# Windere/EAS-SNN

Measured on AMD Instinct MI355X. Metric: event-frames/sec (T=3) SYOLOX-S Gen1 304x240, higher is better.
Workload: dtype f32

## Files before the change

eas_snn_amd/_ctx.py:

```python
import os


def _env_flag(name, default='1'):
    return os.environ.get(name, default) == '1'


class Context:
    def __init__(self):
        self.spike_planes = _env_flag('EAS_SPIKE_PLANES')
        self.conv_stats = _env_flag('EAS_CONV_STATS')
        self.conv_stats_max_blocks = int(os.environ.get('EAS_CONV_STATS_MAX_BLOCKS', '4096'))
        self.fused_eval = {'1': 'all', 'all': 'all', '0': False, 'auto': 'auto'}.get(os.environ.get('EAS_FUSED_EVAL', 'auto'), 'auto')
        self.fused_ann_eval = _env_flag('EAS_FUSED_ANN_EVAL')
        self.arsnn_fused = _env_flag('EAS_ARSNN_FUSED')
        self.small_dgrad = os.environ.get('EAS_SMALL_DGRAD', '1') != '0'
        self.defer_wgrad_reduce = _env_flag('EAS_DEFER_WGRAD_REDUCE', '0')
        self.wgrad_side_batch = int(os.environ.get('EAS_WGRAD_SIDE', '16'))
        self.dwconv = _env_flag('EAS_DWCONV')
        self.device_ap = _env_flag('EAS_DEVICE_AP')
        self.verify_small_int = False
        self.state_writeback = True
        self.planes_scope = False
        self.invstd_scope = None
        self.want_conv_stats = False
        self.conv_stats_slot = None
        self.replicas = 1
        self.pack_scope = None
        self.pack_gen = 0
        self.frozen = None
        self.pending_reduce = []
        self.side = {'stream': None, 'pending': [], 'keep': [], 'dirty': False}
        self.deferred_counters = None
        self.call_log = None
        self.timer = None
        self.tag = None
        self.conv_sink = None


ctx = Context()
```

eas_snn_amd/_lib.py:

```python
import ctypes as C
import os
import subprocess

_HERE = os.path.dirname(os.path.abspath(__file__))
LIB_PATH = os.environ.get('EAS_LIB') or os.path.join(_HERE, 'libeas_hip.so')
CSRC = os.path.join(_HERE, 'csrc')

_lib = None

_f32p, _i32p, _u32p, _u16p, _u8p, _i64p, _f64p = (C.c_void_p,) * 7
_P = C.c_void_p

class EasWgradReduceJob(C.Structure):
    _fields_ = [('slabs', C.c_void_p), ('grad_w', C.c_void_p), ('n', C.c_int), ('slabs_count', C.c_int)]


class EasSmallconvPackJob(C.Structure):
    _fields_ = [('w', C.c_void_p), ('wr', C.c_void_p), ('Cin', C.c_int), ('Cout', C.c_int), ('k', C.c_int), ('mode', C.c_int),
                ('o_total', C.c_int), ('o_off', C.c_int)]


class EasBnPending(C.Structure):
    _fields_ = [('partial', C.c_void_p), ('chunks', C.c_int), ('replicas', C.c_int), ('count', C.c_double), ('eps', C.c_float),
                ('momentum', C.c_float), ('running_mean', C.c_void_p), ('running_var', C.c_void_p), ('pitch', C.c_int)]


class EasLifRange(C.Structure):
    _fields_ = [('gamma', C.c_void_p), ('beta', C.c_void_p), ('mean', C.c_void_p), ('invstd', C.c_void_p), ('w_logit', C.c_void_p),
                ('k_const', C.c_float), ('v_th', C.c_float), ('planes', C.c_void_p), ('out_f32', C.c_void_p), ('out_ctot', C.c_int),
                ('out_c0', C.c_int), ('res_planes', C.c_void_p), ('res_f32', C.c_void_p), ('res_ctot', C.c_int), ('rate', C.c_void_p),
                ('v_in', C.c_void_p), ('v_out', C.c_void_p)]


class EasConvBnLifEval(C.Structure):
    _fields_ = [('x', C.c_void_p), ('packed_w', C.c_void_p), ('x_terms', C.c_int), ('x_shared', C.c_int), ('T', C.c_int), ('N', C.c_int),
                ('Cin', C.c_int), ('Cout', C.c_int), ('Hi', C.c_int), ('Wi', C.c_int), ('ksize', C.c_int), ('stride', C.c_int),
                ('csplit', C.c_int), ('range', EasLifRange * 2)]


class EasBnActRange(C.Structure):
    _fields_ = [('gamma', C.c_void_p), ('beta', C.c_void_p), ('mean', C.c_void_p), ('invstd', C.c_void_p), ('out', C.c_void_p),
                ('out_ctot', C.c_int), ('out_c0', C.c_int)]


class EasConvBnActEval(C.Structure):
    _fields_ = [('x', C.c_void_p), ('packed_w', C.c_void_p), ('x_terms', C.c_int), ('NI', C.c_int), ('Cin', C.c_int), ('Cout', C.c_int),
                ('Hi', C.c_int), ('Wi', C.c_int), ('ksize', C.c_int), ('stride', C.c_int), ('act', C.c_int), ('csplit', C.c_int),
                ('range', EasBnActRange * 2)]


class EasConvProblem(C.Structure):
    _fields_ = [('x', C.c_void_p), ('packed_w', C.c_void_p), ('bias', C.c_void_p), ('y', C.c_void_p), ('stats', C.c_void_p),
                ('NI', C.c_int), ('Cin', C.c_int), ('Cout', C.c_int), ('Hi', C.c_int), ('Wi', C.c_int), ('accumulate', C.c_int)]


class EasBnSiluFwdProblem(C.Structure):
    _fields_ = [('y', C.c_void_p), ('mean', C.c_void_p), ('invstd', C.c_void_p), ('gamma', C.c_void_p), ('beta', C.c_void_p),
                ('out', C.c_void_p), ('N', C.c_int), ('C', C.c_int), ('HW', C.c_int), ('out_ctot', C.c_int), ('y_ctot', C.c_int),
                ('pending', EasBnPending)]


class EasBnSiluBwdProblem(C.Structure):
    _fields_ = [('grad_out', C.c_void_p), ('y', C.c_void_p), ('mean', C.c_void_p), ('invstd', C.c_void_p), ('gamma', C.c_void_p),
                ('beta', C.c_void_p), ('grad_y', C.c_void_p), ('grad_gamma', C.c_void_p), ('grad_beta', C.c_void_p),
                ('workspace', C.c_void_p), ('batch_stats', C.c_int), ('N', C.c_int), ('C', C.c_int), ('HW', C.c_int),
                ('grad_out_ctot', C.c_int), ('y_ctot', C.c_int)]


class EasWgradProblem(C.Structure):
    _fields_ = [('x', C.c_void_p), ('grad_y', C.c_void_p), ('workspace', C.c_void_p), ('NI', C.c_int), ('Cin', C.c_int), ('Cout', C.c_int),
                ('Hi', C.c_int), ('Wi', C.c_int)]


class EasChannelSumProblem(C.Structure):
    _fields_ = [('g', C.c_void_p), ('out', C.c_void_p), ('N', C.c_int), ('C', C.c_int), ('HW', C.c_int)]


class EasPredDgradProblem(C.Structure):
    _fields_ = [('gy_a', C.c_void_p), ('w_a', C.c_void_p), ('Ka', C.c_int), ('gy_b', C.c_void_p), ('w_b', C.c_void_p), ('Kb', C.c_int),
                ('gx', C.c_void_p), ('N', C.c_int), ('C', C.c_int), ('HW', C.c_int)]


class EasAdamHyper(C.Structure):
    _fields_ = [('beta1', C.c_double), ('beta2', C.c_double), ('eps', C.c_double), ('group_lr', C.c_double * 16), ('ema_updates', C.c_void_p),
                ('ema_decay', C.c_double), ('ema_ramp', C.c_double)]


ABI_VERSION = 9

PROTOTYPES = {
    'eas_abi_version': (C.c_int, []),
    'eas_kernel_trace_begin': (None, []),
    'eas_kernel_trace_dump': (C.c_int64, [C.c_char_p, C.c_int64]),
    'eas_launch_counter': (C.c_int64, []),
    'eas_status_string': (C.c_char_p, [C.c_int]),
    'eas_conv_bn_lif_eval': (C.c_int, [C.POINTER(EasConvBnLifEval), _P]),
    'eas_conv_bn_lif_eval_supported': (C.c_int, [C.c_int] * 10),
    'eas_conv_bn_act_eval': (C.c_int, [C.POINTER(EasConvBnActEval), _P, _P]),
    'eas_conv_bn_act_eval_group': (C.c_int, [C.POINTER(EasConvBnActEval), C.c_int, _P]),
    'eas_event_histogram': (C.c_int, [_P, _P, _P, _P, C.c_int64, _P, C.c_int, C.c_int, C.c_int, C.c_int, _P, _P, _P]),
    'eas_event_histogram_dat': (C.c_int, [_P, C.c_int64, _P, C.c_int, C.c_int, C.c_int, C.c_int, _P, _P, _P]),
    'eas_counts_to_canvas': (C.c_int, [_P, C.c_int64, C.c_int, C.c_int, C.c_int, C.c_int, _P, _P]),
    'eas_event_voxel_cube': (C.c_int, [_P, _P, _P, _P, C.c_int64, _P, C.c_int, C.c_int, C.c_int, C.c_int, C.c_int, _P, _P]),
    'eas_event_time_surface': (C.c_int, [_P, _P, _P, _P, C.c_int64, _P, C.c_int, C.c_int, C.c_int, C.c_int, C.c_double, _P, _P, _P]),
    'eas_spike_sop_workspace_doubles': (C.c_int64, []),
    'eas_spike_sop': (C.c_int, [_P, C.c_int64, C.c_int, C.c_int, C.c_int, C.c_int, C.c_int, C.c_int, _P, _P, _P]),
    'eas_counts_letterbox': (C.c_int, [_P, _P, C.c_int, C.c_int, C.c_int, C.c_int, C.c_int, C.c_int, _P, _P]),
    'eas_postprocess_workspace_bytes': (C.c_int64, [C.c_int, C.c_int]),
    'eas_postprocess': (C.c_int, [_P, C.c_int, C.c_int, C.c_int, C.c_float, C.c_float, C.c_int, _P, _P, _P, _P]),
    'eas_event_frames': (C.c_int, [_P, _P, _P, _P, C.c_int64, _P, C.c_int, C.c_int, C.c_int, C.c_int, C.c_int, C.c_int, _P, _P, _P, _P]),
    'eas_simota_assign': (C.c_int, [_P] * 8 + [C.c_int] * 4 + [_P] * 4),
    'eas_simota_assign_rows': (C.c_int, [_P] * 6 + [C.c_int] * 4 + [_P] * 4),
    'eas_det_decode': (C.c_int, [C.c_int, _P, _P, _P, _P, _P, C.c_int, C.c_int, _P, _P]),
    'eas_det_decode_eval': (C.c_int, [C.c_int, _P, _P, _P, _P, _P, C.c_int, C.c_int, _P, _P]),
    'eas_det_labels': (C.c_int, [_P, C.c_int, C.c_int, _P, _P, _P, _P, _P]),
    'eas_det_loss_workspace_doubles': (C.c_int64, []),
    'eas_det_loss': (C.c_int, [C.c_int] + [_P] * 8 + [C.c_int, C.c_int] + [_P] * 3 + [C.c_int] + [_P] * 4 + [C.c_int, _P, _P, _P]),
    'eas_upcat_fwd': (C.c_int, [_P, _P, _P, C.c_int64] + [C.c_int] * 5 + [_P]),
    'eas_upcat_bwd': (C.c_int, [_P, _P, _P, C.c_int64] + [C.c_int] * 5 + [_P]),
    'eas_upcat_planes_fwd': (C.c_int, [_P, _P, _P, C.c_int64] + [C.c_int] * 5 + [_P]),
    'eas_focus': (C.c_int, [_P, _P, C.c_int64, C.c_int, C.c_int, C.c_int, C.c_int, _P]),
    'eas_event_voxel_grid': (C.c_int, [_P, _P, _P, _P, C.c_int64, _P, C.c_int, C.c_int, C.c_int, C.c_int, _P, _P]),
    'eas_event_window_search': (C.c_int, [_P, _P, C.c_int, _P, _P, C.c_int, C.c_int64, C.c_int64, C.c_int, _P, _P]),
    'eas_event_histogram_dat_ranges': (C.c_int, [_P, _P] + [C.c_int] * 4 + [_P, _P, _P]),
    'eas_stacked_hist_event_sum': (C.c_int, [_P, _P] + [C.c_int] * 7 + [_P, _P]),
    'eas_lif_fwd': (C.c_int, [_P, _P, _P, _P, C.c_float, C.c_float, C.c_float, C.c_int, _P, _P, _P, C.c_int, C.c_int64, _P]),
    'eas_lif_bwd': (C.c_int, [_P, _P, _P, _P, _P, _P, C.c_float, C.c_float, C.c_float, C.c_int, C.c_int, C.c_float,
                              _P, _P, _P, C.c_int, C.c_int64, _P]),
    'eas_lif_bwd_patan': (C.c_int, [_P, _P, _P, _P, _P, _P, C.c_float, C.c_float, C.c_float, C.c_int, _P, _P,
                                    _P, _P, _P, C.c_int, C.c_int64, _P]),
    'eas_reduce_workspace_floats': (C.c_int64, [C.c_int64]),
    'eas_time_mean': (C.c_int, [_P, _P, C.c_int, C.c_int64, _P]),
    'eas_channel_sum': (C.c_int, [_P, _P, C.c_int, C.c_int, C.c_int, _P]),
    'eas_bn_stats': (C.c_int, [_P, C.c_int, C.c_int, C.c_int, C.c_int, C.c_float, C.c_float, _P, _P, _P, _P, _P, _P]),
    'eas_bn_workspace_doubles': (C.c_int64, [C.c_int]),
    'eas_bn_lif_fwd': (C.c_int, [_P, _P, _P, _P, _P, _P, _P, _P, C.c_float, C.c_float, C.c_float, C.c_int, _P, _P,
                                 C.c_int, C.c_int, C.c_int, C.c_int, C.c_int, _P]),
    'eas_bn_lif_bwd': (C.c_int, [_P, _P, _P, _P, _P, _P, _P, _P, _P, C.c_float, C.c_float, C.c_float, C.c_int, C.c_int,
                                 C.c_float, C.c_int, _P, _P, _P, _P, _P, C.c_int, C.c_int, C.c_int, C.c_int, C.c_int, _P]),
    'eas_bn_silu_fwd': (C.c_int, [_P] * 6 + [C.c_int] * 3 + [_P]),
    'eas_bn_silu_fwd_ex': (C.c_int, [_P] * 6 + [C.c_int] * 3 + [C.POINTER(EasBnPending), C.c_int, C.c_int, _P]),
    'eas_bn_stats_partial': (C.c_int, [_P, C.c_int, C.c_int, C.c_int, C.c_int, _P, _P]),
    'eas_bn_lif_fwd_ex': (C.c_int, [_P, C.c_int, _P, _P, _P, _P, _P, _P, _P, C.c_float, C.c_float, C.c_float, C.c_int, _P, _P,
                                    C.c_int, C.c_int, C.c_int, C.c_int, C.c_int, C.POINTER(EasBnPending), _P, C.c_int, _P, _P, C.c_int, _P]),
    'eas_bn_lif_bwd_ex': (C.c_int, [_P, C.c_int, _P, _P, C.c_int, _P, _P, _P, _P, _P, _P, C.c_float, C.c_float, C.c_float, C.c_int, C.c_int,
                                    C.c_float, C.c_int, _P, _P, _P, _P, _P, C.c_int, C.c_int, C.c_int, C.c_int, C.c_int, _P]),
    'eas_bn_lif_bwd_patan': (C.c_int, [_P, C.c_int, _P, _P, C.c_int, _P, _P, _P, _P, _P, _P, C.c_float, C.c_float, C.c_float, C.c_int, _P,
                                       _P, C.c_int, _P, _P, _P, _P, _P, C.c_int, C.c_int, C.c_int, C.c_int, C.c_int, _P]),
    'eas_bn_silu_bwd': (C.c_int, [_P] * 6 + [C.c_int] + [_P] * 4 + [C.c_int] * 5 + [_P]),
    'eas_arsnn_step_fwd': (C.c_int, [_P] * 14 + [C.c_int, C.c_int, C.c_int, C.c_int, C.c_float, C.c_float, C.c_int,
                                                 C.c_int, C.c_int, C.c_int, _P]),
    'eas_arsnn_step_bwd': (C.c_int, [_P] * 13 + [C.c_int, C.c_int, C.c_int, C.c_int, C.c_float, C.c_float, C.c_int,
                                                 C.c_float, C.c_int, C.c_int, C.c_int, _P]),
    'eas_arsnn_tail_fwd': (C.c_int, [_P] * 6 + [C.c_int] * 7 + [_P]),
    'eas_arsnn_tail_bwd': (C.c_int, [_P] * 6 + [C.c_int] * 7 + [_P]),
    'eas_arsnn_fused_step_fwd': (C.c_int, [_P] * 19 + [C.c_int, C.c_int, C.c_int, C.c_int, C.c_float, C.c_float, C.c_int,
                                                       C.c_int, C.c_int, C.c_int, C.c_int, _P]),
    'eas_smallconv_packed_floats': (C.c_int64, [C.c_int] * 3),
    'eas_smallconv_pack_weights': (C.c_int, [_P, C.c_int, _P]),
    'eas_smallconv_bwd_input_dual': (C.c_int, [_P] * 6 + [C.c_int] * 4 + [_P]),
    'eas_smallconv_fwd': (C.c_int, [_P] * 4 + [C.c_int] * 8 + [_P]),
    'eas_smallconv_bwd_input': (C.c_int, [_P] * 4 + [C.c_int] * 6 + [_P]),
    'eas_smallconv_bwd_weight': (C.c_int, [_P] * 5 + [C.c_int] * 7 + [_P]),
    'eas_smallconv_wgrad_workspace_floats': (C.c_int64, [C.c_int] * 3),
    'eas_conv_packed_weight_bytes': (C.c_int64, [C.c_int] * 4),
    'eas_conv_pack_weights': (C.c_int, [_P, _P] + [C.c_int] * 4 + [_P]),
    'eas_conv_pack_weights_many': (C.c_int, [_P, C.c_int, _P]),
    'eas_conv_fwd_supported': (C.c_int, [C.c_int] * 8),
    'eas_conv_wgrad_parts': (C.c_int, [C.c_int] * 7),
    'eas_conv_fwd': (C.c_int, [_P] * 4 + [C.c_int] * 8 + [_P, _P]),
    'eas_conv_fwd_act': (C.c_int, [_P] * 4 + [C.c_int] * 9 + [_P, _P]),
    'eas_conv_fwd_planes': (C.c_int, [_P] * 4 + [C.c_int] * 7 + [_P, C.c_int, _P]),
    'eas_spike_planes_from_f32': (C.c_int, [_P, C.c_int, _P, C.c_int, C.c_int64, C.c_int, C.c_int, _P, _P]),
    'eas_spike_planes_to_f32': (C.c_int, [_P, C.c_int, _P, C.c_int, C.c_int64, C.c_int, C.c_int, _P]),
    'eas_conv_fwd_stats': (C.c_int, [_P] * 3 + [C.c_int] * 8 + [_P, _P, C.c_int, _P]),
    'eas_conv_fwd_stats_blocks': (C.c_int, [C.c_int] * 8),
    'eas_conv_dgrad_s2': (C.c_int, [_P] * 3 + [C.c_int] * 5 + [_P]),
    'eas_conv_dgrad_small_supported': (C.c_int, [C.c_int] * 5),
    'eas_conv_dgrad_small': (C.c_int, [_P] * 3 + [C.c_int] * 5 + [_P]),
    'eas_conv_wgrad_workspace_floats': (C.c_int64, [C.c_int] * 8),
    'eas_conv_wgrad': (C.c_int, [_P] * 4 + [C.c_int] * 8 + [_P]),
    'eas_conv_wgrad_partial': (C.c_int, [_P] * 3 + [C.c_int] * 8 + [_P]),
    'eas_conv_wgrad_planes_partial': (C.c_int, [_P] * 3 + [C.c_int] * 7 + [_P]),
    'eas_conv_wgrad_reduce_many': (C.c_int, [_P, C.c_int, _P]),
    'eas_dwconv_supported': (C.c_int, [C.c_int] * 6),
    'eas_dwconv_fwd_stats_blocks': (C.c_int, [C.c_int] * 6),
    'eas_dwconv_fwd': (C.c_int, [_P] * 4 + [C.c_int] * 5 + [_P, C.c_int, _P]),
    'eas_dwconv_fwd_planes': (C.c_int, [_P] * 4 + [C.c_int] * 5 + [_P, C.c_int, _P]),
    'eas_dwconv_dgrad': (C.c_int, [_P] * 3 + [C.c_int] * 5 + [_P]),
    'eas_dwconv_wgrad_workspace_floats': (C.c_int64, [C.c_int] * 5),
    'eas_dwconv_wgrad': (C.c_int, [_P] * 4 + [C.c_int] * 5 + [_P]),
    'eas_dwconv_wgrad_planes': (C.c_int, [_P] * 4 + [C.c_int] * 5 + [_P]),
    'eas_spp_pool_fwd': (C.c_int, [_P, _P, C.c_int64] + [C.c_int] * 6 + [_P]),
    'eas_spp_pool_bwd': (C.c_int, [_P, _P, _P, C.c_int64] + [C.c_int] * 6 + [_P]),
    'eas_spp_pool_planes_fwd': (C.c_int, [_P, _P, C.c_int64] + [C.c_int] * 6 + [_P]),
    'eas_spp_pool_planes_bwd': (C.c_int, [_P, _P, _P, C.c_int64] + [C.c_int] * 6 + [_P]),
    'eas_conv_fwd_group_plan': (C.c_int, [C.POINTER(EasConvProblem), C.c_int, C.c_int, C.c_int, C.POINTER(C.c_int)]),
    'eas_conv_fwd_group': (C.c_int, [C.POINTER(EasConvProblem), C.c_int, C.c_int, C.c_int, _P]),
    'eas_bn_silu_fwd_group': (C.c_int, [C.POINTER(EasBnSiluFwdProblem), C.c_int, _P]),
    'eas_bn_silu_bwd_group': (C.c_int, [C.POINTER(EasBnSiluBwdProblem), C.c_int, _P]),
    'eas_conv_wgrad_group_plan': (C.c_int, [C.POINTER(EasWgradProblem), C.c_int, C.c_int, C.c_int, C.POINTER(C.c_int)]),
    'eas_conv_wgrad_group_partial': (C.c_int, [C.POINTER(EasWgradProblem), C.c_int, C.c_int, C.c_int, _P]),
    'eas_channel_sum_group': (C.c_int, [C.POINTER(EasChannelSumProblem), C.c_int, _P]),
    'eas_pred_dgrad_group': (C.c_int, [C.POINTER(EasPredDgradProblem), C.c_int, _P]),
    'eas_adam_table_entry_bytes': (C.c_int, []),
    'eas_adam_chunk': (C.c_int, []),
    'eas_adam_step': (C.c_int, [_P, C.c_int, C.c_longlong, C.c_double, C.c_double, C.c_double, _P]),
    'eas_adam_advance_steps': (C.c_int, [_P, C.c_int, _P]),
    'eas_adam_step_ex': (C.c_int, [_P, C.c_int, C.c_longlong, C.POINTER(EasAdamHyper), _P]),
    'eas_adam_advance_steps_ex': (C.c_int, [_P, C.c_int, _P, _P]),
    'eas_cocoeval_supported': (C.c_int, [C.c_int64] * 3 + [C.c_int] * 5 + [C.c_int64]),
    'eas_cocoeval_workspace_bytes': (C.c_int64, [C.c_int64]),
    'eas_cocoeval_keys': (C.c_int, [_P, _P, _P, C.c_int64, _P, _P, C.c_int64, C.c_int64, C.c_int, _P, _P, _P]),
    'eas_cocoeval_match': (C.c_int, [_P, _P, _P, C.c_int64, _P, _P, _P, _P, C.c_int64, C.c_int64, C.c_int, _P, C.c_int, _P, C.c_int, C.c_int,
                                     C.c_int64, _P, _P, _P, _P, _P, _P]),
    'eas_cocoeval_accumulate': (C.c_int, [_P] * 5 + [C.c_int64, _P, C.c_int, C.c_int, _P, C.c_int, C.c_int, _P, C.c_int, _P, _P, _P, _P]),
}


class EasHipError(RuntimeError):
    pass


def build(verbose=False):
    cmd = ['make', '-C', CSRC, '-j', str(min(8, os.cpu_count() or 1))]
    r = subprocess.run(cmd, stdout=subprocess.PIPE, stderr=subprocess.STDOUT, text=True)
    if verbose or r.returncode != 0:
        print(r.stdout)
    if r.returncode != 0:
        raise EasHipError('building libeas_hip.so failed')
    return LIB_PATH


def _bind_host_hip_runtime():
    import torch
    cand = os.path.join(os.path.dirname(torch.__file__), 'lib', 'libamdhip64.so')
    if not os.path.exists(cand):
        cand = 'libamdhip64.so'
    C.CDLL(cand, mode=C.RTLD_GLOBAL)


_PRIVATE_STREAMS = []


def private_stream():
    import torch
    _bind_host_hip_runtime()
    rt = C.CDLL(None)
    handle = C.c_void_p()
    rc = rt.hipStreamCreateWithFlags(C.byref(handle), C.c_uint(1))
    if rc != 0 or not handle.value:
        raise EasHipError(f'hipStreamCreateWithFlags failed ({rc})')
    st = torch.cuda.ExternalStream(handle.value)
    _PRIVATE_STREAMS.append(st)
    return st


def lib():
    global _lib
    if _lib is None:
        if not os.path.exists(LIB_PATH):
            raise EasHipError(
                f'{LIB_PATH} is missing: the HIP extension has not been built and eas_snn_amd has no CPU fallback. '
                'Run `python -c "import __graft_entry__ as g; g.build()"`.')
        _bind_host_hip_runtime()
        handle = C.CDLL(LIB_PATH)
        for name, (res, args) in PROTOTYPES.items():
            fn = getattr(handle, name)
            fn.restype = res
            fn.argtypes = args
        if handle.eas_abi_version() != ABI_VERSION:
            raise EasHipError('libeas_hip.so ABI version mismatch; rebuild')
        _lib = handle
    return _lib


def check(status, what):
    if status != 0:
        msg = lib().eas_status_string(status).decode()
        raise EasHipError(f'{what}: status {status} ({msg})')


def ptr(t):
    return None if t is None else t.data_ptr()


_RAW_STREAM = None


def stream():
    global _RAW_STREAM
    if _RAW_STREAM is None:
        import torch
        raw = getattr(torch._C, '_cuda_getCurrentRawStream', None)
        if raw is not None:
            _RAW_STREAM = lambda: raw(torch.cuda.current_device())
        else:
            _RAW_STREAM = lambda: torch.cuda.current_stream().cuda_stream
    return _RAW_STREAM()
```

eas_snn_amd/csrc/arsnn.hip:

```cpp
#include "eas_common.h"
#include "smallconv_core.h"

namespace {

constexpr int VEC = 4;

typedef int8_t eas_state_t;
__device__ __forceinline__ int4 load_q8(const eas_state_t* p) {
    const int w = *reinterpret_cast<const int*>(p);
    return make_int4((int)(int8_t)(w & 0xFF), (int)(int8_t)((w >> 8) & 0xFF), (int)(int8_t)((w >> 16) & 0xFF), (int)(int8_t)((w >> 24) & 0xFF));
}
__device__ __forceinline__ void store_q8(eas_state_t* p, const int4& v) {
    *reinterpret_cast<int*>(p) = (v.x & 0xFF) | ((v.y & 0xFF) << 8) | ((v.z & 0xFF) << 16) | ((v.w & 0xFF) << 24);
}

struct StepCfg {
    int t, Ts, readout, spike_attach, soft_reset;
    float thresh, v_reset, sg_alpha;
    int64_t plane;
    int64_t total;
};

__device__ __forceinline__ void step_elem(float g_in, float c_in, float g_rec, float c_rec, float v, float vsum,
                                          int32_t& seg, int32_t& tl, float* __restrict__ agg, int64_t i,
                                          const StepCfg& c, float& v_out, float& vsum_out, float& spike, float& gate,
                                          float& vn) {
    gate = eas_sigmoidf(g_in + g_rec);
    const float cur = c_in + c_rec;
    vn = gate * v + cur;
    spike = (vn - c.thresh) > 0.0f ? 1.0f : 0.0f;
    v_out = c.soft_reset ? vn - c.thresh * spike : vn * (1.0f - spike) + c.v_reset * spike;
    const float vs1 = vsum + vn;
    if (spike != 0.0f) {
        if (c.readout != 3 && seg < c.Ts) {
            float val = c.readout == 0 ? vs1 : (c.readout == 1 ? v_out : vs1 / (float)(c.t - tl));
            if (c.spike_attach) val = val * spike;
            agg[(int64_t)seg * c.total + i] += val;
            seg += 1;
            tl = c.t;
        }
        vsum_out = c.readout == 3 ? vs1 : 0.0f;
    } else {
        vsum_out = vs1;
    }
}

__global__ __launch_bounds__(EAS_BLOCK) void arsnn_step_fwd_kernel(
    const float* __restrict__ conv_in, const float* __restrict__ conv_rec, const float* __restrict__ v,
    const float* __restrict__ vsum, eas_state_t* __restrict__ seg, eas_state_t* __restrict__ t_last, float* __restrict__ agg,
    float* __restrict__ v_out, float* __restrict__ vsum_out, float* __restrict__ spike_out,
    float* __restrict__ gate_save, float* __restrict__ vn_save, eas_state_t* __restrict__ seg_before,
    eas_state_t* __restrict__ tl_before, StepCfg c) {
    const int64_t ngroups = c.total / VEC;
    for (int64_t g = (int64_t)blockIdx.x * blockDim.x + threadIdx.x; g < ngroups; g += (int64_t)gridDim.x * blockDim.x) {
        const int64_t i = g * VEC;
        const int64_t n = i / c.plane;
        const int64_t r = i - n * c.plane;
        const int64_t cb = n * 2 * c.plane + r;
        const float4 gi = *reinterpret_cast<const float4*>(conv_in + cb);
        const float4 ci = *reinterpret_cast<const float4*>(conv_in + cb + c.plane);
        const float4 gr = *reinterpret_cast<const float4*>(conv_rec + cb);
        const float4 cr = *reinterpret_cast<const float4*>(conv_rec + cb + c.plane);
        float4 vv = make_float4(0.f, 0.f, 0.f, 0.f), vs = vv;
        int4 sg = make_int4(0, 0, 0, 0), tl = make_int4(-1, -1, -1, -1);
        if (v) {
            vv = *reinterpret_cast<const float4*>(v + i);
            vs = *reinterpret_cast<const float4*>(vsum + i);
            sg = load_q8(seg + i);
            tl = load_q8(t_last + i);
        }
        if (seg_before) store_q8(seg_before + i, sg);
        if (tl_before) store_q8(tl_before + i, tl);
        float4 vo, vso, sp, ga, vn;
        step_elem(gi.x, ci.x, gr.x, cr.x, vv.x, vs.x, sg.x, tl.x, agg, i + 0, c, vo.x, vso.x, sp.x, ga.x, vn.x);
        step_elem(gi.y, ci.y, gr.y, cr.y, vv.y, vs.y, sg.y, tl.y, agg, i + 1, c, vo.y, vso.y, sp.y, ga.y, vn.y);
        step_elem(gi.z, ci.z, gr.z, cr.z, vv.z, vs.z, sg.z, tl.z, agg, i + 2, c, vo.z, vso.z, sp.z, ga.z, vn.z);
        step_elem(gi.w, ci.w, gr.w, cr.w, vv.w, vs.w, sg.w, tl.w, agg, i + 3, c, vo.w, vso.w, sp.w, ga.w, vn.w);
        *reinterpret_cast<float4*>(v_out + i) = vo;
        *reinterpret_cast<float4*>(vsum_out + i) = vso;
        *reinterpret_cast<float4*>(spike_out + i) = sp;
        store_q8(seg + i, sg);
        store_q8(t_last + i, tl);
        if (gate_save) *reinterpret_cast<float4*>(gate_save + i) = ga;
        if (vn_save) *reinterpret_cast<float4*>(vn_save + i) = vn;
    }
}

template <int K, bool HAS_G>
__global__ __launch_bounds__(NT, 2) void arsnn_fused_step_fwd_kernel(
    const float* __restrict__ a_in, const float* __restrict__ wr_in, const float* __restrict__ b_in, const float* __restrict__ a_g,
    const float* __restrict__ wr_g, const float* __restrict__ b_g, const float* __restrict__ r_const, const float* __restrict__ v,
    const float* __restrict__ vsum, eas_state_t* __restrict__ seg, eas_state_t* __restrict__ t_last, float* __restrict__ agg,
    float* __restrict__ v_out, float* __restrict__ vsum_out, float* __restrict__ spike_out, float* __restrict__ gate_save,
    float* __restrict__ vn_save, eas_state_t* __restrict__ seg_before, eas_state_t* __restrict__ tl_before, StepCfg c, int N, int H, int W) {
    using SG = Stage<4, K, true>;
    constexpr int LWF = SG::PITCH, PLANE = SG::PLANE;
    using St = typename SG::St;
    St st;
    st.init(H, W);
    __shared__ __attribute__((aligned(16))) float lds[4 * PLANE];
    const int tiles_x = (W + TW - 1) / TW, tiles_y = (H + TH - 1) / TH;
    const int ntiles = N * tiles_x * tiles_y;
    const int tx = threadIdx.x & 15, ty = threadIdx.x >> 4;
    const int HW = H * W;
    float4 pre[St::PER];
    unsigned okm = 0;
    int tile = blockIdx.x;
    if (tile < ntiles)
        okm = st.load(a_in, pre, tile / (tiles_x * tiles_y), H, W, ((tile / tiles_x) % tiles_y) * TH, (tile % tiles_x) * TW);
    for (; tile < ntiles; tile += gridDim.x) {
        const int n = tile / (tiles_x * tiles_y);
        const int ty0 = ((tile / tiles_x) % tiles_y) * TH, tx0 = (tile % tiles_x) * TW;
        const int nxt = tile + gridDim.x;
        __syncthreads();
        st.store(lds, pre, okm);
        __syncthreads();
        if (HAS_G) okm = st.load(a_g, pre, n, H, W, ty0, tx0);
        else if (nxt < ntiles) okm = st.load(a_in, pre, nxt / (tiles_x * tiles_y), H, W, ((nxt / tiles_x) % tiles_y) * TH, (nxt % tiles_x) * TW);
        const int oy = ty0 + ty, ox = tx0 + 4 * tx;
        const bool inside = oy < H && ox < W;
        const int pix = oy * W + ox;
        float4 vv[2], vs[2], rg[2], rcur[2];
        int4 sg[2], tl[2];
#pragma unroll
        for (int c2 = 0; c2 < 2; ++c2) {
            vv[c2] = make_float4(0.f, 0.f, 0.f, 0.f); vs[c2] = vv[c2]; rg[c2] = vv[c2]; rcur[c2] = vv[c2];
            sg[c2] = make_int4(0, 0, 0, 0); tl[c2] = make_int4(-1, -1, -1, -1);
            if (inside) {
                const int64_t i = ((int64_t)n * 2 + c2) * HW + pix;
                if (v) {
                    vv[c2] = *reinterpret_cast<const float4*>(v + i);
                    vs[c2] = *reinterpret_cast<const float4*>(vsum + i);
                    sg[c2] = load_q8(seg + i);
                    tl[c2] = load_q8(t_last + i);
                }
                if (!HAS_G && r_const) {
                    rg[c2] = *reinterpret_cast<const float4*>(r_const + (int64_t)c2 * HW + pix);
                    rcur[c2] = *reinterpret_cast<const float4*>(r_const + (int64_t)(2 + c2) * HW + pix);
                }
            }
        }
        __builtin_amdgcn_sched_barrier(0);
        f2 X[4][2], R[4][2];
#pragma unroll
        for (int op = 0; op < 2; ++op) {
            const f2 bx = b_in ? f2{b_in[2 * op], b_in[2 * op + 1]} : f2{0.f, 0.f};
            const f2 bg = (HAS_G && b_g) ? f2{b_g[2 * op], b_g[2 * op + 1]} : f2{0.f, 0.f};
#pragma unroll
            for (int j = 0; j < 4; ++j) { X[j][op] = bx; R[j][op] = bg; }
        }
        sc_accumulate<4, 4, K, LWF, SG::NQ, SG::OFS>(lds, PLANE, wr_in, X, tx, ty);
        if (HAS_G) {
            __syncthreads();
            st.store(lds, pre, okm);
            __syncthreads();
            if (nxt < ntiles) okm = st.load(a_in, pre, nxt / (tiles_x * tiles_y), H, W, ((nxt / tiles_x) % tiles_y) * TH, (nxt % tiles_x) * TW);
            sc_accumulate<4, 4, K, LWF, SG::NQ, SG::OFS>(lds, PLANE, wr_g, R, tx, ty);
        }
        if (inside) {
#pragma unroll
            for (int c2 = 0; c2 < 2; ++c2) {
                float gi[4], ci[4], gr[4], cr[4];
#pragma unroll
                for (int j = 0; j < 4; ++j) {
                    gi[j] = c2 ? X[j][0].y : X[j][0].x;
                    ci[j] = c2 ? X[j][1].y : X[j][1].x;
                    gr[j] = c2 ? R[j][0].y : R[j][0].x;
                    cr[j] = c2 ? R[j][1].y : R[j][1].x;
                }
                if (!HAS_G && r_const) {
                    gr[0] = rg[c2].x; gr[1] = rg[c2].y; gr[2] = rg[c2].z; gr[3] = rg[c2].w;
                    cr[0] = rcur[c2].x; cr[1] = rcur[c2].y; cr[2] = rcur[c2].z; cr[3] = rcur[c2].w;
                }
                const int64_t i = ((int64_t)n * 2 + c2) * HW + pix;
                if (seg_before) store_q8(seg_before + i, sg[c2]);
                if (tl_before) store_q8(tl_before + i, tl[c2]);
                float4 vo, vso, sp, ga, vn;
                step_elem(gi[0], ci[0], gr[0], cr[0], vv[c2].x, vs[c2].x, sg[c2].x, tl[c2].x, agg, i + 0, c, vo.x, vso.x, sp.x, ga.x, vn.x);
                step_elem(gi[1], ci[1], gr[1], cr[1], vv[c2].y, vs[c2].y, sg[c2].y, tl[c2].y, agg, i + 1, c, vo.y, vso.y, sp.y, ga.y, vn.y);
                step_elem(gi[2], ci[2], gr[2], cr[2], vv[c2].z, vs[c2].z, sg[c2].z, tl[c2].z, agg, i + 2, c, vo.z, vso.z, sp.z, ga.z, vn.z);
                step_elem(gi[3], ci[3], gr[3], cr[3], vv[c2].w, vs[c2].w, sg[c2].w, tl[c2].w, agg, i + 3, c, vo.w, vso.w, sp.w, ga.w, vn.w);
                *reinterpret_cast<float4*>(v_out + i) = vo;
                *reinterpret_cast<float4*>(vsum_out + i) = vso;
                *reinterpret_cast<float4*>(spike_out + i) = sp;
                store_q8(seg + i, sg[c2]);
                store_q8(t_last + i, tl[c2]);
                if (gate_save) *reinterpret_cast<float4*>(gate_save + i) = ga;
                if (vn_save) *reinterpret_cast<float4*>(vn_save + i) = vn;
            }
        }
    }
}

__device__ __forceinline__ void step_elem_bwd(float gv_out, float gvs_out, float gsp, const float* __restrict__ g_agg,
                                              int64_t i, float v_prev, float vsum_prev, float gate, float vn, int32_t seg_b,
                                              int32_t tl_b, const StepCfg& c, float& g_gatepre, float& g_cur,
                                              float& g_v_prev, float& g_vsum_prev) {
    const float spike = (vn - c.thresh) > 0.0f ? 1.0f : 0.0f;
    const bool fired = spike != 0.0f;
    const float vs1 = vsum_prev + vn;
    float d_vs1 = (fired && c.readout != 3) ? 0.0f : gvs_out;
    float d_vout = gv_out;
    float d_s = gsp;
    if (fired && c.readout != 3 && seg_b < c.Ts) {
        const float ga = g_agg[(int64_t)seg_b * c.total + i];
        float d_pre = ga;
        if (c.spike_attach) {
            const float v_out = c.soft_reset ? vn - c.thresh : c.v_reset;
            const float pre = c.readout == 0 ? vs1 : (c.readout == 1 ? v_out : vs1 / (float)(c.t - tl_b));
            d_s += ga * pre;
            d_pre = ga * spike;
        }
        if (c.readout == 0) d_vs1 += d_pre;
        else if (c.readout == 1) d_vout += d_pre;
        else d_vs1 += d_pre / (float)(c.t - tl_b);
    }
    float d_vn = d_vs1;
    g_vsum_prev = d_vs1;
    if (c.soft_reset) {
        d_vn += d_vout;
        d_s += d_vout * (-c.thresh);
    } else {
        d_vn += d_vout * (1.0f - spike);
        d_s += d_vout * (c.v_reset - vn);
    }
    d_vn += d_s * eas_surrogate_grad(EAS_SG_RECT, c.sg_alpha, vn - c.thresh);
    g_cur = d_vn;
    g_v_prev = d_vn * gate;
    g_gatepre = (d_vn * v_prev) * gate * (1.0f - gate);
}

__global__ __launch_bounds__(EAS_BLOCK) void arsnn_step_bwd_kernel(
    const float* __restrict__ g_v_out, const float* __restrict__ g_vsum_out, const float* __restrict__ g_spike,
    const float* __restrict__ g_agg, const float* __restrict__ v_prev, const float* __restrict__ vsum_prev,
    const float* __restrict__ gate_save, const float* __restrict__ vn_save, const eas_state_t* __restrict__ seg_before,
    const eas_state_t* __restrict__ tl_before, float* __restrict__ g_conv, float* __restrict__ g_v_prev,
    float* __restrict__ g_vsum_prev, StepCfg c) {
    for (int64_t i = (int64_t)blockIdx.x * blockDim.x + threadIdx.x; i < c.total; i += (int64_t)gridDim.x * blockDim.x) {
        const int64_t n = i / c.plane;
        const int64_t r = i - n * c.plane;
        const int64_t cb = n * 2 * c.plane + r;
        float gg, gc, gvp, gvsp;
        step_elem_bwd(g_v_out ? g_v_out[i] : 0.f, g_vsum_out ? g_vsum_out[i] : 0.f, g_spike ? g_spike[i] : 0.f, g_agg, i,
                      v_prev ? v_prev[i] : 0.f, vsum_prev ? vsum_prev[i] : 0.f, gate_save[i], vn_save[i], seg_before[i], tl_before[i], c, gg, gc,
                      gvp, gvsp);
        g_conv[cb] = gg;
        g_conv[cb + c.plane] = gc;
        g_v_prev[i] = gvp;
        g_vsum_prev[i] = gvsp;
    }
}

__global__ __launch_bounds__(EAS_BLOCK) void arsnn_tail_fwd_kernel(const float* __restrict__ v, const float* __restrict__ vsum,
                                                                   const float* __restrict__ spike_last,
                                                                   const eas_state_t* __restrict__ seg,
                                                                   const eas_state_t* __restrict__ t_last, float* __restrict__ agg,
                                                                   int Tm, int Ts, int readout, int write_zero, int64_t total) {
    for (int64_t i = (int64_t)blockIdx.x * blockDim.x + threadIdx.x; i < total; i += (int64_t)gridDim.x * blockDim.x) {
        if (spike_last[i] != 0.0f) continue;
        const int s = seg[i];
        if (s >= Ts) continue;
        float val = readout == 0 ? vsum[i] : (readout == 1 ? v[i] : vsum[i] / (float)(Tm - 1 - t_last[i]));
        if (write_zero) val = val * 0.0f;
        agg[(int64_t)s * total + i] += val;
    }
}

__global__ __launch_bounds__(EAS_BLOCK) void arsnn_tail_bwd_kernel(const float* __restrict__ g_agg,
                                                                   const float* __restrict__ spike_last,
                                                                   const eas_state_t* __restrict__ seg,
                                                                   const eas_state_t* __restrict__ t_last, float* __restrict__ g_v,
                                                                   float* __restrict__ g_vsum, int Tm, int Ts, int readout,
                                                                   int write_zero, int64_t total) {
    for (int64_t i = (int64_t)blockIdx.x * blockDim.x + threadIdx.x; i < total; i += (int64_t)gridDim.x * blockDim.x) {
        float gv = 0.f, gvs = 0.f;
        const int s = seg[i];
        if (spike_last[i] == 0.0f && s < Ts && !write_zero) {
            const float ga = g_agg[(int64_t)s * total + i];
            if (readout == 0) gvs = ga;
            else if (readout == 1) gv = ga;
            else gvs = ga / (float)(Tm - 1 - t_last[i]);
        }
        g_v[i] = gv;
        g_vsum[i] = gvs;
    }
}

}

extern "C" {

int eas_arsnn_step_fwd(const float* conv_in, const float* conv_rec, const float* v, const float* vsum,
                       int8_t* seg, int8_t* t_last, float* agg, float* v_out, float* vsum_out, float* spike_out,
                       float* gate_save, float* vn_save, int8_t* seg_before, int8_t* t_last_before, int t,
                       int Ts, int readout, int spike_attach, float thresh, float v_reset, int soft_reset, int N,
                       int C2, int HW, eas_stream_t stream) {
    if (!conv_in || !conv_rec || (v == nullptr) != (vsum == nullptr) || !seg || !t_last || !agg || !v_out || !vsum_out || !spike_out)
        return EAS_ERR_INVALID_ARG;
    if (N < 1 || C2 < 1 || HW < 1 || Ts < 1 || t < 0 || readout < 0 || readout > 3) return EAS_ERR_INVALID_ARG;
    if (HW % VEC != 0 || Ts > 127 || t > 126) return EAS_ERR_UNSUPPORTED;
    if (((uintptr_t)conv_in | (uintptr_t)conv_rec | (uintptr_t)v | (uintptr_t)vsum | (uintptr_t)seg | (uintptr_t)t_last |
         (uintptr_t)v_out | (uintptr_t)vsum_out | (uintptr_t)spike_out | (uintptr_t)gate_save | (uintptr_t)vn_save |
         (uintptr_t)seg_before | (uintptr_t)t_last_before) & 15)
        return EAS_ERR_INVALID_ARG;
    StepCfg c{t, Ts, readout, spike_attach, soft_reset, thresh, v_reset, 1.0f, (int64_t)C2 * HW, (int64_t)N * C2 * HW};
    EAS_CLEAR_ERR();
    EAS_LAUNCH(arsnn_step_fwd_kernel, dim3(eas_grid_1d(c.total / VEC)), dim3(EAS_BLOCK), 0, eas_s(stream), conv_in,
                       conv_rec, v, vsum, seg, t_last, agg, v_out, vsum_out, spike_out, gate_save, vn_save, seg_before,
                       t_last_before, c);
    EAS_CHECK_LAUNCH();
    return EAS_OK;
}

int eas_arsnn_fused_step_fwd(const float* a_in, const float* wr_in, const float* b_in, const float* a_g, const float* wr_g, const float* b_g,
                             const float* r_const, const float* v, const float* vsum, int8_t* seg, int8_t* t_last, float* agg, float* v_out,
                             float* vsum_out, float* spike_out, float* gate_save, float* vn_save, int8_t* seg_before, int8_t* t_last_before,
                             int t, int Ts, int readout, int spike_attach, float thresh, float v_reset, int soft_reset, int N, int H, int W, int k,
                             eas_stream_t stream) {
    if (!a_in || !wr_in || (a_g && !wr_g) || (v == nullptr) != (vsum == nullptr) || !seg || !t_last || !agg || !v_out || !vsum_out || !spike_out)
        return EAS_ERR_INVALID_ARG;
    if (N < 1 || H < 1 || W < 1 || Ts < 1 || t < 0 || readout < 0 || readout > 3) return EAS_ERR_INVALID_ARG;
    if (W % 4 != 0 || (k != 3 && k != 5 && k != 7) || Ts > 127 || t > 126) return EAS_ERR_UNSUPPORTED;
    if (((uintptr_t)a_in | (uintptr_t)a_g | (uintptr_t)wr_in | (uintptr_t)wr_g | (uintptr_t)r_const | (uintptr_t)v | (uintptr_t)vsum | (uintptr_t)seg | (uintptr_t)t_last |
         (uintptr_t)v_out | (uintptr_t)vsum_out | (uintptr_t)spike_out | (uintptr_t)gate_save | (uintptr_t)vn_save | (uintptr_t)seg_before |
         (uintptr_t)t_last_before) & 15)
        return EAS_ERR_INVALID_ARG;
    const int HW = H * W;
    StepCfg c{t, Ts, readout, spike_attach, soft_reset, thresh, v_reset, 1.0f, (int64_t)2 * HW, (int64_t)N * 2 * HW};
    int tiles = N * ((H + TH - 1) / TH) * ((W + TW - 1) / TW);
    if (tiles > 256 * 6) tiles = 256 * 6;
    hipStream_t st = eas_s(stream);
    EAS_CLEAR_ERR();
#define EAS_FUSED(K_)                                                                                                                        \
    do {                                                                                                                                     \
        if (a_g)                                                                                                                             \
            EAS_LAUNCH((arsnn_fused_step_fwd_kernel<K_, true>), dim3(tiles), dim3(NT), 0, st, a_in, wr_in, b_in, a_g, wr_g, b_g,     \
                               r_const, v, vsum, seg, t_last, agg, v_out, vsum_out, spike_out, gate_save, vn_save, seg_before,               \
                               t_last_before, c, N, H, W);                                                                                    \
        else                                                                                                                                 \
            EAS_LAUNCH((arsnn_fused_step_fwd_kernel<K_, false>), dim3(tiles), dim3(NT), 0, st, a_in, wr_in, b_in, a_g, wr_g, b_g,    \
                               r_const, v, vsum, seg, t_last, agg, v_out, vsum_out, spike_out, gate_save, vn_save, seg_before,               \
                               t_last_before, c, N, H, W);                                                                                    \
    } while (0)
    if (k == 3) EAS_FUSED(3);
    else if (k == 5) EAS_FUSED(5);
    else EAS_FUSED(7);
#undef EAS_FUSED
    EAS_CHECK_LAUNCH();
    return EAS_OK;
}

int eas_arsnn_step_bwd(const float* g_v_out, const float* g_vsum_out, const float* g_spike, const float* g_agg,
                       const float* v_prev, const float* vsum_prev, const float* gate_save, const float* vn_save,
                       const int8_t* seg_before, const int8_t* t_last_before, float* g_conv, float* g_v_prev,
                       float* g_vsum_prev, int t, int Ts, int readout, int spike_attach, float thresh,
                       float v_reset, int soft_reset, float sg_alpha, int N, int C2, int HW, eas_stream_t stream) {
    if (!g_agg || (v_prev == nullptr) != (vsum_prev == nullptr) || !gate_save || !vn_save || !seg_before || !t_last_before || !g_conv ||
        !g_v_prev || !g_vsum_prev)
        return EAS_ERR_INVALID_ARG;
    if (N < 1 || C2 < 1 || HW < 1 || Ts < 1 || t < 0 || readout < 0 || readout > 3 || !(sg_alpha > 0.f))
        return EAS_ERR_INVALID_ARG;
    StepCfg c{t, Ts, readout, spike_attach, soft_reset, thresh, v_reset, sg_alpha, (int64_t)C2 * HW,
              (int64_t)N * C2 * HW};
    EAS_CLEAR_ERR();
    EAS_LAUNCH(arsnn_step_bwd_kernel, dim3(eas_grid_1d(c.total)), dim3(EAS_BLOCK), 0, eas_s(stream), g_v_out,
                       g_vsum_out, g_spike, g_agg, v_prev, vsum_prev, gate_save, vn_save, seg_before, t_last_before, g_conv,
                       g_v_prev, g_vsum_prev, c);
    EAS_CHECK_LAUNCH();
    return EAS_OK;
}

int eas_arsnn_tail_fwd(const float* v, const float* vsum, const float* spike_last, const int8_t* seg,
                       const int8_t* t_last, float* agg, int Tm, int Ts, int readout, int write_zero, int N,
                       int C2, int HW, eas_stream_t stream) {
    if (!v || !vsum || !spike_last || !seg || !t_last || !agg || N < 1 || C2 < 1 || HW < 1 || Ts < 1 || readout < 0 ||
        readout > 2)
        return EAS_ERR_INVALID_ARG;
    const int64_t total = (int64_t)N * C2 * HW;
    EAS_CLEAR_ERR();
    EAS_LAUNCH(arsnn_tail_fwd_kernel, dim3(eas_grid_1d(total)), dim3(EAS_BLOCK), 0, eas_s(stream), v, vsum,
                       spike_last, seg, t_last, agg, Tm, Ts, readout, write_zero, total);
    EAS_CHECK_LAUNCH();
    return EAS_OK;
}

int eas_arsnn_tail_bwd(const float* g_agg, const float* spike_last, const int8_t* seg, const int8_t* t_last,
                       float* g_v, float* g_vsum, int Tm, int Ts, int readout, int write_zero, int N, int C2,
                       int HW, eas_stream_t stream) {
    if (!g_agg || !spike_last || !seg || !t_last || !g_v || !g_vsum || N < 1 || C2 < 1 || HW < 1 || Ts < 1 ||
        readout < 0 || readout > 2)
        return EAS_ERR_INVALID_ARG;
    const int64_t total = (int64_t)N * C2 * HW;
    EAS_CLEAR_ERR();
    EAS_LAUNCH(arsnn_tail_bwd_kernel, dim3(eas_grid_1d(total)), dim3(EAS_BLOCK), 0, eas_s(stream), g_agg, spike_last,
                       seg, t_last, g_v, g_vsum, Tm, Ts, readout, write_zero, total);
    EAS_CHECK_LAUNCH();
    return EAS_OK;
}

}
```

eas_snn_amd/csrc/smallconv_wgrad_mfma.hip:

```cpp
#include "eas_common.h"

namespace {

typedef __bf16 bf16x8 __attribute__((ext_vector_type(8)));
typedef float f32x16 __attribute__((ext_vector_type(16)));
typedef unsigned int u32x4 __attribute__((ext_vector_type(4)));

constexpr int RB = 8;
constexpr int WC = 64;
constexpr int HALO = 8;
constexpr int XC = WC + 2 * HALO;
constexpr int NTH = 256;
constexpr int NWV = NTH / 64;

template <int CIN, int COUT, int K>
struct Sw {
    static constexpr int PAD = K / 2;
    static constexpr int GR = RB + K - 1;
    static constexpr int GP = WC + 8;
    static constexpr int G_ROWS = GR * COUT;
    static constexpr int G_TERM = G_ROWS * GP * 2;
    static constexpr int XP = XC;
    static constexpr int X_ROWS = RB * CIN;
    static constexpr int X_RAW = (X_ROWS + 1) * XP * 2;
    static constexpr int X_COPY = X_RAW + ((4 + 32 - (X_RAW / 4) % 32) % 32) * 4;
    static constexpr int X_ONES = X_ROWS * XP * 2 + 8;
    static constexpr int X_TERM = 2 * X_COPY;
    static constexpr int G_BYTES = 3 * G_TERM;
    static constexpr int X_BYTES = 3 * X_TERM;
    static constexpr int STAGE_BYTES = G_BYTES + X_BYTES;
    static constexpr int RED_BYTES = 2 * NWV * 32 * 33 * 4;
    static constexpr int LDS_BYTES = STAGE_BYTES > RED_BYTES ? STAGE_BYTES : RED_BYTES;
    static constexpr int NWT = COUT * CIN * K * K;
    static constexpr int NOUT = NWT + COUT;
    static constexpr int G_ITEMS = GR * COUT * (WC / 8);
    static constexpr int X_ITEMS = RB * CIN * (XC / 8);
    static_assert(COUT * K <= 32 && CIN * K + 1 <= 32, "does not fit one 32x32 tile");
    static_assert(PAD + 1 <= HALO && XC <= XP && (X_COPY / 4) % 32 == 4 && X_COPY % 16 == 0, "x staging geometry");
    static_assert(2 * STAGE_BYTES <= 160 * 1024 && STAGE_BYTES % 16 == 0, "LDS");
    static_assert(RB == 2 * NWV, "two rows per wave (4 waves) / one row per wave (8 waves)");
};

__device__ __forceinline__ void sw_split3(float v, __bf16& hi, __bf16& mid, __bf16& lo) {
    hi = (__bf16)v;
    const float r1 = v - (float)hi;
    mid = (__bf16)r1;
    lo = (__bf16)(r1 - (float)mid);
}

template <int O, int NV>
__device__ __forceinline__ void sw_store_terms(unsigned char* dst, int term_stride, const float (&v)[NV]) {
    bf16x8 t0, t1, t2;
#pragma unroll
    for (int j = 0; j < 8; ++j) {
        __bf16 a, b, c;
        sw_split3(v[O + j], a, b, c);
        t0[j] = a;
        t1[j] = b;
        t2[j] = c;
    }
    *(bf16x8*)dst = t0;
    *(bf16x8*)(dst + term_stride) = t1;
    *(bf16x8*)(dst + 2 * term_stride) = t2;
}

template <int NV>
__device__ __forceinline__ void sw_load_row(const float* __restrict__ row, bool row_ok, int c0, int W, float (&v)[NV]) {
#pragma unroll
    for (int j = 0; j < NV; ++j) {
        const int c = c0 + j;
        v[j] = (row_ok && c >= 0 && c < W) ? row[c] : 0.f;
    }
}

template <int CIN, int COUT, int K, bool VEC>
__global__ __launch_bounds__(VEC ? 4 * NTH : NTH) void smallconv_wgrad_mfma_kernel(const float* __restrict__ gy, const float* __restrict__ x,
                                                                                   float* __restrict__ partial, int N, int H, int W, int x_tm) {
    using S = Sw<CIN, COUT, K>;
    const int xS = x_tm ? N / x_tm : 0;
    auto x_img = [&](int n) {
        if (x_tm == 0) return n;
        const int t = n / xS;
        return (n - t * xS) * x_tm + (x_tm - 1 - t);
    };
    constexpr int PAD = S::PAD;
    constexpr int NBUF = VEC ? 2 : 1;
    extern __shared__ __attribute__((aligned(16))) unsigned char smem[];
    const int tid = threadIdx.x, lane = tid & 63;
    constexpr int NTS = VEC ? 2 * NTH : NTH;
    constexpr int NCW = VEC ? 2 * NWV : NWV;
    constexpr int RPW = RB / NCW;
    const int wave = VEC ? (tid >> 6) - NTS / 64 : (tid >> 6);
    const int r = lane & 31, hh = lane >> 5;

    const bool g0 = (r & 3) == r || (r >= 12 && r < 16) || (r >= 20 && r < 28);
    const int ra = r < COUT * K ? r : (g0 ? 0 : 4);
    const int a_kh = ra / COUT, a_co = ra % COUT;
    const int a_off = (((2 * PAD - a_kh) * COUT + a_co) * S::GP + 8 * hh) * 2;
    const int a_rs = COUT * S::GP * 2, a_kss = 32;
    const bool b_ones = r == CIN * K;
    const int rb = r < CIN * K ? r : 0;
    const int b_ci = rb / K, b_kw = rb % K;
    const int sft = b_kw - PAD;
    const int odd = sft & 1;
    const int b_off = b_ones ? S::X_ONES : odd * S::X_COPY + (b_ci * S::XP + HALO + 8 * hh + (sft - odd)) * 2;
    const int b_rs = b_ones ? 0 : CIN * S::XP * 2, b_kss = b_ones ? 0 : 32;

    for (int i = tid; i < NBUF * 3 * 4; i += blockDim.x) {
        const int buf = i / 12, tm = (i % 12) / 4, d = i & 3;
        *(unsigned int*)(smem + buf * S::STAGE_BYTES + S::G_BYTES + tm * S::X_TERM + S::X_ONES + 4 * d) = tm == 0 ? 0x3f803f80u : 0u;
    }

    f32x16 acc0, acc1;
#pragma unroll
    for (int e = 0; e < 16; ++e) {
        acc0[e] = 0.0f;
        acc1[e] = 0.0f;
    }

    const int bands = (H + RB - 1) / RB, chunks = (W + WC - 1) / WC;
    const int ntiles = N * bands * chunks;
    const size_t plane = (size_t)H * W;

    auto tile_origin = [&](int t, int& n, int& h0, int& w0) {
        n = t / (bands * chunks);
        const int rest = t - n * bands * chunks;
        const int band = rest / chunks;
        h0 = band * RB;
        w0 = (rest - band * chunks) * WC;
    };

    struct Frag { bf16x8 a[3], b[3]; };
    const unsigned char* pa0 = smem + a_off + wave * a_rs;
    const unsigned char* pb0 = smem + S::G_BYTES + b_off + wave * b_rs;
    auto read_frag = [&](Frag& f, int step) {
        const int ks = step / RPW, i = step % RPW;
        const unsigned char* pa = pa0 + i * (NCW * a_rs) + ks * a_kss;
        const unsigned char* pb = pb0 + i * (NCW * b_rs) + ks * b_kss;
#pragma unroll
        for (int tm = 0; tm < 3; ++tm) {
            f.a[tm] = *(const bf16x8*)(pa + tm * S::G_TERM);
            const unsigned int* q = (const unsigned int*)(pb + tm * S::X_TERM);
            u32x4 d;
            d[0] = q[0]; d[1] = q[1]; d[2] = q[2]; d[3] = q[3];
            f.b[tm] = __builtin_bit_cast(bf16x8, d);
        }
    };
    auto mul6 = [&](f32x16& acc, const Frag& f) {
        acc = __builtin_amdgcn_mfma_f32_32x32x16_bf16(f.a[2], f.b[0], acc, 0, 0, 0);
        acc = __builtin_amdgcn_mfma_f32_32x32x16_bf16(f.a[0], f.b[2], acc, 0, 0, 0);
        acc = __builtin_amdgcn_mfma_f32_32x32x16_bf16(f.a[1], f.b[1], acc, 0, 0, 0);
        acc = __builtin_amdgcn_mfma_f32_32x32x16_bf16(f.a[1], f.b[0], acc, 0, 0, 0);
        acc = __builtin_amdgcn_mfma_f32_32x32x16_bf16(f.a[0], f.b[1], acc, 0, 0, 0);
        acc = __builtin_amdgcn_mfma_f32_32x32x16_bf16(f.a[0], f.b[0], acc, 0, 0, 0);
    };
    auto compute = [&](int buf) {
        constexpr int STEPS = RPW * (WC / 16);
        pa0 = smem + buf * S::STAGE_BYTES + a_off + wave * a_rs;
        pb0 = smem + buf * S::STAGE_BYTES + S::G_BYTES + b_off + wave * b_rs;
        Frag f0, f1;
        read_frag(f0, 0);
#pragma unroll
        for (int st = 0; st < STEPS; st += 2) {
            read_frag(f1, st + 1);
            mul6(acc0, f0);
            if (st + 2 < STEPS) read_frag(f0, st + 2);
            mul6(acc1, f1);
        }
    };

    auto write_red = [&]() {
        float* red = (float*)smem;
#pragma unroll
        for (int e = 0; e < 16; ++e) {
            const int m = 4 * hh + (e & 3) + 8 * (e >> 2);
            red[(wave * 32 + m) * 33 + r] = acc0[e] + acc1[e];
        }
    };

    if constexpr (VEC) {
        constexpr int NG = (S::G_ITEMS + NTS - 1) / NTS, NX = (S::X_ITEMS + NTS - 1) / NTS;
        int g_dr[NG], g_dc[NG], g_ch[NG], g_lds[NG];
        int x_dr[NX], x_dc[NX], x_ch[NX], x_lds[NX];
        bool g_valid[NG], x_valid[NX];
#pragma unroll
        for (int j = 0; j < NG; ++j) {
            const int id = j * NTS + tid;
            g_valid[j] = tid < NTS && id < S::G_ITEMS;
            const int idc = g_valid[j] ? id : 0;
            const int c8 = idc % (WC / 8), rc = idc / (WC / 8);
            const int co = rc % COUT, jrow = rc / COUT;
            g_dr[j] = jrow - PAD; g_dc[j] = 8 * c8; g_ch[j] = co;
            g_lds[j] = ((jrow * COUT + co) * S::GP + 8 * c8) * 2;
        }
#pragma unroll
        for (int j = 0; j < NX; ++j) {
            const int id = j * NTS + (((j + NG) & 1) ? NTS - 1 - tid : tid);
            x_valid[j] = tid < NTS && id >= 0 && id < S::X_ITEMS;
            const int idc = x_valid[j] ? id : 0;
            const int c8 = idc % (XC / 8), rc = idc / (XC / 8);
            const int ci = rc % CIN, row_l = rc / CIN;
            x_dr[j] = row_l; x_dc[j] = 8 * c8 - HALO; x_ch[j] = ci;
            x_lds[j] = S::G_BYTES + ((row_l * CIN + ci) * S::XP + 8 * c8) * 2;
        }
        struct Pre {
            float4 ga[NG], gb[NG], xa[NX], xb[NX];
            float xc[NX];
            int gm[NG], xm[NX];
        };
        auto issue = [&](Pre& p, int t) {
            int n, h0, w0;
            tile_origin(t, n, h0, w0);
            const int nx = x_img(n);
#pragma unroll
            for (int j = 0; j < NG; ++j) {
                const int row = h0 + g_dr[j], col = w0 + g_dc[j];
                const bool row_ok = g_valid[j] && (unsigned)row < (unsigned)H;
                const bool ok0 = row_ok && col + 4 <= W, ok1 = row_ok && col + 8 <= W;
                const float* prow = gy + ((size_t)n * COUT + g_ch[j]) * plane + (size_t)(row_ok ? row : 0) * W + col;
                p.ga[j] = *(const float4*)(ok0 ? prow : gy);
                p.gb[j] = *(const float4*)(ok1 ? prow + 4 : gy);
                p.gm[j] = (ok0 ? 1 : 0) | (ok1 ? 2 : 0);
            }
#pragma unroll
            for (int j = 0; j < NX; ++j) {
                const int row = h0 + x_dr[j], col = w0 + x_dc[j];
                const bool row_ok = x_valid[j] && row < H;
                const bool ok0 = row_ok && col >= 0 && col + 4 <= W, ok1 = row_ok && col + 4 >= 0 && col + 8 <= W;
                const bool ok2 = row_ok && col + 8 < W;
                const float* prow = x + ((size_t)nx * CIN + x_ch[j]) * plane + (size_t)(row_ok ? row : 0) * W + col;
                p.xa[j] = *(const float4*)(ok0 ? prow : x);
                p.xb[j] = *(const float4*)(ok1 ? prow + 4 : x);
                p.xc[j] = *(ok2 ? prow + 8 : x);
                p.xm[j] = (ok0 ? 1 : 0) | (ok1 ? 2 : 0) | (ok2 ? 4 : 0);
            }
        };
        auto commit = [&](const Pre& p, int buf) {
            unsigned char* const base = smem + buf * S::STAGE_BYTES;
#pragma unroll
            for (int j = 0; j < NG; ++j) {
                if (!g_valid[j]) continue;
                const bool ok0 = p.gm[j] & 1, ok1 = p.gm[j] & 2;
                float v[8];
                v[0] = ok0 ? p.ga[j].x : 0.f; v[1] = ok0 ? p.ga[j].y : 0.f; v[2] = ok0 ? p.ga[j].z : 0.f; v[3] = ok0 ? p.ga[j].w : 0.f;
                v[4] = ok1 ? p.gb[j].x : 0.f; v[5] = ok1 ? p.gb[j].y : 0.f; v[6] = ok1 ? p.gb[j].z : 0.f; v[7] = ok1 ? p.gb[j].w : 0.f;
                sw_store_terms<0, 8>(base + g_lds[j], S::G_TERM, v);
            }
#pragma unroll
            for (int j = 0; j < NX; ++j) {
                if (!x_valid[j]) continue;
                const bool ok0 = p.xm[j] & 1, ok1 = p.xm[j] & 2, ok2 = p.xm[j] & 4;
                float v[9];
                v[0] = ok0 ? p.xa[j].x : 0.f; v[1] = ok0 ? p.xa[j].y : 0.f; v[2] = ok0 ? p.xa[j].z : 0.f; v[3] = ok0 ? p.xa[j].w : 0.f;
                v[4] = ok1 ? p.xb[j].x : 0.f; v[5] = ok1 ? p.xb[j].y : 0.f; v[6] = ok1 ? p.xb[j].z : 0.f; v[7] = ok1 ? p.xb[j].w : 0.f;
                v[8] = ok2 ? p.xc[j] : 0.f;
                unsigned char* dst = base + x_lds[j];
                sw_store_terms<0, 9>(dst, S::X_TERM, v);
                sw_store_terms<1, 9>(dst + S::X_COPY, S::X_TERM, v);
            }
        };
        const int G = gridDim.x;
        const bool stager = __builtin_amdgcn_readfirstlane(tid >> 6) < NTS / 64;
        int t = blockIdx.x;
        if (stager) {
            Pre pa, pb;
            issue(pa, t);
            if (t + G < ntiles) issue(pb, t + G);
            commit(pa, 0);
            if (t + 2 * G < ntiles) issue(pa, t + 2 * G);
            __syncthreads();
            for (;;) {
                if (t + G < ntiles) {
                    commit(pb, 1);
                    if (t + 3 * G < ntiles) issue(pb, t + 3 * G);
                }
                __syncthreads();
                t += G;
                if (t >= ntiles) break;
                if (t + G < ntiles) {
                    commit(pa, 0);
                    if (t + 3 * G < ntiles) issue(pa, t + 3 * G);
                }
                __syncthreads();
                t += G;
                if (t >= ntiles) break;
            }
        } else {
            __syncthreads();
            for (;;) {
                compute(0);
                __syncthreads();
                t += G;
                if (t >= ntiles) break;
                compute(1);
                __syncthreads();
                t += G;
                if (t >= ntiles) break;
            }
            write_red();
        }
    } else {
        __syncthreads();
        for (int t = blockIdx.x; t < ntiles; t += gridDim.x) {
            int n, h0, w0;
            tile_origin(t, n, h0, w0);
            for (int id = tid; id < S::G_ITEMS; id += NTH) {
                const int c8 = id % (WC / 8), rc = id / (WC / 8);
                const int co = rc % COUT, jrow = rc / COUT;
                const int ho = h0 - PAD + jrow;
                const bool row_ok = ho >= 0 && ho < H;
                const float* row = gy + ((size_t)n * COUT + co) * plane + (size_t)(row_ok ? ho : 0) * W;
                float v[8];
                sw_load_row<8>(row, row_ok, w0 + 8 * c8, W, v);
                sw_store_terms<0, 8>(smem + ((jrow * COUT + co) * S::GP + 8 * c8) * 2, S::G_TERM, v);
            }
            for (int id = tid; id < S::X_ITEMS; id += NTH) {
                const int c8 = id % (XC / 8), rc = id / (XC / 8);
                const int ci = rc % CIN, row_l = rc / CIN;
                const int h = h0 + row_l;
                const bool row_ok = h < H;
                const float* row = x + ((size_t)x_img(n) * CIN + ci) * plane + (size_t)(row_ok ? h : 0) * W;
                float v[9];
                sw_load_row<9>(row, row_ok, w0 - HALO + 8 * c8, W, v);
                unsigned char* dst = smem + S::G_BYTES + ((row_l * CIN + ci) * S::XP + 8 * c8) * 2;
                sw_store_terms<0, 9>(dst, S::X_TERM, v);
                sw_store_terms<1, 9>(dst + S::X_COPY, S::X_TERM, v);
            }
            __syncthreads();
            compute(0);
            __syncthreads();
        }
        write_red();
    }

    const float* red = (const float*)smem;
    __syncthreads();
    for (int e = tid; e < S::NOUT; e += blockDim.x) {
        int m, nn;
        if (e < S::NWT) {
            const int co = e / (CIN * K * K), rem = e % (CIN * K * K);
            const int ci = rem / (K * K), kk = rem % (K * K);
            m = (kk / K) * COUT + co;
            nn = ci * K + kk % K;
        } else {
            m = PAD * COUT + (e - S::NWT);
            nn = CIN * K;
        }
        float s = 0.f;
#pragma unroll
        for (int wv = 0; wv < NCW; ++wv) s += red[(wv * 32 + m) * 33 + nn];
        partial[(int64_t)blockIdx.x * S::NOUT + e] = s;
    }
}

template <int CIN, int COUT, int K>
int sw_launch_k(bool vec, const float* gy, const float* x, float* partial, int nblocks, int N, int H, int W, int x_tm, hipStream_t st) {
    using S = Sw<CIN, COUT, K>;
    if (vec) {
        auto kern = smallconv_wgrad_mfma_kernel<CIN, COUT, K, true>;
        static bool attr_set = false;
        if (!attr_set) {
            if (hipFuncSetAttribute((const void*)kern, hipFuncAttributeMaxDynamicSharedMemorySize, 160 * 1024) != hipSuccess) return EAS_ERR_LAUNCH;
            attr_set = true;
        }
        EAS_LAUNCH(kern, dim3(nblocks), dim3(4 * NTH), 2 * S::STAGE_BYTES, st, gy, x, partial, N, H, W, x_tm);
    } else {
        EAS_LAUNCH((smallconv_wgrad_mfma_kernel<CIN, COUT, K, false>), dim3(nblocks), dim3(NTH), S::LDS_BYTES, st, gy, x, partial, N, H, W, x_tm);
    }
    return EAS_OK;
}

template <int CIN, int COUT>
int sw_launch(int k, const float* gy, const float* x, float* partial, int nblocks, int N, int H, int W, int x_tm, hipStream_t st) {
    const bool vec = (W & 3) == 0 && ((((uintptr_t)gy) | ((uintptr_t)x)) & 15) == 0;
    int rc;
    if (vec && nblocks > 256) nblocks = 256;
    switch (k) {
        case 3: rc = sw_launch_k<CIN, COUT, 3>(vec, gy, x, partial, nblocks, N, H, W, x_tm, st); break;
        case 5: rc = sw_launch_k<CIN, COUT, 5>(vec, gy, x, partial, nblocks, N, H, W, x_tm, st); break;
        case 7: rc = sw_launch_k<CIN, COUT, 7>(vec, gy, x, partial, nblocks, N, H, W, x_tm, st); break;
        default: return EAS_ERR_UNSUPPORTED;
    }
    if (rc != EAS_OK) return rc;
    EAS_CHECK_LAUNCH();
    return nblocks;
}

}

int eas_sw_mfma_partials(const float* gy, const float* x, float* partial, int max_blocks, int N, int Cin, int Cout, int H, int W,
                         int k, int x_tm, hipStream_t st) {
    const int64_t tiles = (int64_t)N * ((H + RB - 1) / RB) * ((W + WC - 1) / WC);
    if (tiles > 0x7fffffff) return EAS_ERR_UNSUPPORTED;
    const int nblocks = tiles < max_blocks ? (int)tiles : max_blocks;
    int rc;
    if (Cin == 2 && Cout == 4) rc = sw_launch<2, 4>(k, gy, x, partial, nblocks, N, H, W, x_tm, st);
    else if (Cin == 4 && Cout == 4) rc = sw_launch<4, 4>(k, gy, x, partial, nblocks, N, H, W, x_tm, st);
    else if (Cin == 2 && Cout == 2) rc = sw_launch<2, 2>(k, gy, x, partial, nblocks, N, H, W, x_tm, st);
    else return EAS_ERR_UNSUPPORTED;
    return rc;
}
```

eas_snn_amd/ops.py:

```python
import sys
import types

from . import ops_bn, ops_conv, ops_core, ops_dwconv, ops_lif, ops_sampler
from ._ctx import ctx

_PLUMBING = {'C', 'collections', 'os', 'torch', '_lib', 'check', 'ptr', 'stream', 'opctx'}
for _m in (ops_core, ops_lif, ops_bn, ops_sampler, ops_dwconv, ops_conv):
    for _k, _v in vars(_m).items():
        if not _k.startswith('__') and _k not in _PLUMBING:
            globals()[_k] = _v
from ._lib import check, ptr, stream

from .ops_events import *
from .ops_glue import *
from .ops_det import *

_ALIASES = {
    '_STATE_WRITEBACK': 'state_writeback', '_TIMER': 'timer', '_TAG': 'tag', '_CALL_LOG': 'call_log', 'SPIKE_PLANES': 'spike_planes',
    '_PLANES_SCOPE': 'planes_scope', '_INVSTD_SCOPE': 'invstd_scope', 'CONV_STATS': 'conv_stats', 'CONV_STATS_MAX_BLOCKS': 'conv_stats_max_blocks',
    '_WANT_CONV_STATS': 'want_conv_stats', '_CONV_STATS_SLOT': 'conv_stats_slot', 'FUSED_EVAL': 'fused_eval', '_REPLICAS': 'replicas',
    'ARSNN_FUSED': 'arsnn_fused', 'DEFER_WGRAD_REDUCE': 'defer_wgrad_reduce', '_PENDING_REDUCE': 'pending_reduce',
    'WGRAD_SIDE_BATCH': 'wgrad_side_batch', '_SIDE': 'side',
    'VERIFY_SMALL_INT': 'verify_small_int', 'SMALL_DGRAD': 'small_dgrad', '_PACK_SCOPE': 'pack_scope', '_PACK_GEN': 'pack_gen', '_FROZEN': 'frozen',
    '_CONV_SINK': 'conv_sink', 'FUSED_ANN_EVAL': 'fused_ann_eval', '_DEFERRED': 'deferred_counters', 'DWCONV': 'dwconv',
    'DEVICE_AP': 'device_ap'}


class _OpsModule(types.ModuleType):
    """this module's class: the aliases above as properties, so that ``ops.X`` and ``ops.X = v`` (also ``monkeypatch.setattr(ops, 'X', v)``)
    reach the context object"""


def _alias(field):
    return property(lambda self: getattr(ctx, field), lambda self, value: setattr(ctx, field, value))


for _old, _new in _ALIASES.items():
    assert hasattr(ctx, _new), _new
    setattr(_OpsModule, _old, _alias(_new))
sys.modules[__name__].__class__ = _OpsModule
del _old, _new, _m, _k, _v
```

eas_snn_amd/ops_sampler.py:

```python
import ctypes as C
import os

import torch

from . import _lib
from ._ctx import ctx as opctx
from ._lib import check, ptr, stream
from .ops_core import READOUT_IDS, _call, _dev, _f32c

def smallconv_pack(jobs):
    L = _lib.lib()
    arr = (_lib.EasSmallconvPackJob * len(jobs))()
    outs = []
    for j, (w, mode, o_total, o_off, wr) in enumerate(jobs):
        w = _f32c(w)
        Cout, Cin, k = w.shape[0], w.shape[1], w.shape[-1]
        if wr is None:
            wr = torch.empty(L.eas_smallconv_packed_floats(Cout if mode else Cin, k, o_total), dtype=torch.float32, device=w.device)
        arr[j] = _lib.EasSmallconvPackJob(w.data_ptr(), wr.data_ptr(), Cin, Cout, k, int(mode), int(o_total), int(o_off))
        outs.append(wr)
    check(L.eas_smallconv_pack_weights(arr, len(jobs), stream()), 'eas_smallconv_pack_weights')
    return outs


def smallconv_fwd(x, w, b, relu=False, out=None, wr=None, x_tm=0):
    x = _f32c(x)
    if x_tm:
        assert x.dim() == 5 and x.shape[1] == x_tm
        x = x.view(-1, *x.shape[2:])
    N, Cin, H, W = x.shape
    Cout, k = w.shape[0], w.shape[-1]
    if wr is None:
        wr = smallconv_pack([(w, 0, Cout, 0, None)])[0]
    y = torch.empty((N, Cout, H, W), dtype=torch.float32, device=x.device) if out is None else out
    assert y.is_contiguous() and y.shape == (N, Cout, H, W)
    _call('eas_smallconv_fwd', 4 * (x.numel() + y.numel()), _lib.lib().eas_smallconv_fwd, ptr(x), ptr(wr), ptr(b), ptr(y), N, Cin, Cout,
          H, W, k, int(relu), int(x_tm), stream())
    return y


def smallconv_bwd_input(gy, w, relu_mask=None, out=None, wr=None):
    gy = _f32c(gy)
    N, Cout, H, W = gy.shape
    Cin, k = w.shape[1], w.shape[-1]
    if wr is None:
        wr = smallconv_pack([(w, 1, Cin, 0, None)])[0]
    gx = torch.empty((N, Cin, H, W), dtype=torch.float32, device=gy.device) if out is None else out
    assert gx.is_contiguous() and gx.shape == (N, Cin, H, W)
    _call('eas_smallconv_bwd_input', 4 * (gy.numel() + gx.numel()), _lib.lib().eas_smallconv_bwd_input, ptr(gy), ptr(wr),
          ptr(relu_mask), ptr(gx), N, Cin, Cout, H, W, k, stream())
    return gx


def smallconv_bwd_input_dual(gy, wr8, k, mask_a, mask_b, out_a, out_b):
    gy = _f32c(gy)
    N, C4, H, W = gy.shape
    assert C4 == 4 and out_a.is_contiguous() and out_b.is_contiguous() and out_a.shape == gy.shape == out_b.shape
    _call('eas_smallconv_bwd_input', 4 * 3 * gy.numel(), _lib.lib().eas_smallconv_bwd_input_dual, ptr(gy), ptr(wr8), ptr(mask_a), ptr(mask_b),
          ptr(out_a), ptr(out_b), N, H, W, int(k), stream())


def smallconv_bwd_weight(gy, x, w, x_tm=0):
    gy, x = _f32c(gy), _f32c(x)
    N, Cout, H, W = gy.shape
    assert x.numel() == N * w.shape[1] * H * W and (not x_tm or (x.dim() == 5 and x.shape[1] == x_tm))
    Cin, k = w.shape[1], w.shape[-1]
    L = _lib.lib()
    gw, gb = torch.empty_like(w), torch.empty(Cout, dtype=torch.float32, device=gy.device)
    ws = torch.empty(L.eas_smallconv_wgrad_workspace_floats(Cin, Cout, k), dtype=torch.float32, device=gy.device)
    _call('eas_smallconv_bwd_weight', 4 * (gy.numel() + x.numel()), L.eas_smallconv_bwd_weight, ptr(gy), ptr(x), ptr(gw), ptr(gb),
          ptr(ws), N, Cin, Cout, H, W, k, int(x_tm), stream())
    return gw, gb


def _conv_stack_fwd(x, params, k, mids=None, packs=None):
    ins = []
    n = len(params) // 2
    for i in range(n):
        ins.append(x)
        x = smallconv_fwd(x, params[2 * i], params[2 * i + 1], relu=(i < n - 1), out=mids[i] if mids is not None and i < n - 1 else None,
                          wr=packs[i] if packs is not None else None)
    return x, ins





class _ARSNNFn(torch.autograd.Function):

    @staticmethod
    def forward(ctx, ev, cfg, *params):
        ctx.set_materialize_grads(False)
        _dev(ev, *params)
        L = _lib.lib()
        k, depth, Ts, readout, sat, wz, ab, thresh, v_reset, soft, record, running, d_in, d_gate = cfg[:14]
        ev = _f32c(ev)
        pin, pg = params[:2 * d_in], params[2 * d_in:]
        collated = len(cfg) > 14 and cfg[14]
        v_record = len(cfg) > 15 and cfg[15]
        if collated:
            N, Tm, Cin, H, W = ev.shape
        else:
            Tm, N, Cin, H, W = ev.shape
        HW = H * W
        if HW % 4 != 0:
            raise _lib.EasHipError('sampler needs H*W divisible by 4')
        dev = ev.device
        need_grad = any(ctx.needs_input_grad[2:]) or ctx.needs_input_grad[0]
        st = stream()
        jobs = [(pin[2 * i], 0, pin[2 * i].shape[0], 0, None) for i in range(d_in)] + [(pg[2 * i], 0, pg[2 * i].shape[0], 0, None) for i in range(d_gate)]
        pk = smallconv_pack(jobs) if jobs else []
        pk_in, pk_g = pk[:d_in], pk[d_in:]
        fused = bool(opctx.arsnn_fused and d_in == 2 and d_gate in (0, 2) and W % 4 == 0 and pin[2].shape[:2] == (4, 4) and pin[0].shape[0] == 4
                     and (d_gate == 0 or (pg[2].shape[:2] == (4, 4) and pg[0].shape[0] == 4)) and opctx.conv_sink is None and Tm > 0)
        ctx.in_collated = bool(collated)
        if collated and not (fused and not ctx.needs_input_grad[0]):
            ev = torch.stack([ev[:, Tm - 1 - t] for t in range(Tm)])
            collated = False
        if fused:
            if collated:
                A_in = smallconv_fwd(ev, pin[0], pin[1], relu=True, wr=pk_in[0], x_tm=Tm).view(Tm, N, 4, H, W)
                in_ins = [ev, A_in.view(Tm * N, 4, H, W)]
            else:
                A_in = smallconv_fwd(ev.view(Tm * N, Cin, H, W), pin[0], pin[1], relu=True, wr=pk_in[0]).view(Tm, N, 4, H, W)
                in_ins = [ev.view(Tm * N, Cin, H, W), A_in.view(Tm * N, 4, H, W)]
            X = None
            C2 = 2
        elif d_in:
            X, in_ins = _conv_stack_fwd(ev.view(Tm * N, Cin, H, W), pin, k, packs=pk_in)
            X = X.view(Tm, N, X.shape[1], H, W)
            C2 = X.shape[2] // 2
        else:
            X, in_ins = ev, []
            C2 = X.shape[2] // 2
        shape = (N, C2, H, W)
        v = vsum = None
        if os.environ.get('EAS_ARSNN_ZERO_FILL') == '1':
            v = torch.zeros(shape, device=dev)
            vsum = torch.zeros(shape, device=dev)
        keep = need_grad and d_gate
        fast0 = bool(d_gate) and Tm > 0 and opctx.conv_sink is None and os.environ.get('EAS_ARSNN_STEP0', 'shared') != 'full'
        if keep:
            gate_in = [torch.empty((Tm, N, pg[2 * i].shape[1], H, W), device=dev) for i in range(d_gate)]
            if not fast0:
                gate_in[0][0].zero_()
            spike = gate_in[0][0]
        else:
            gate_in = None
            spike = None if fast0 else torch.zeros(shape, device=dev)
        seg = torch.empty(shape, dtype=torch.int8, device=dev)
        tl = torch.empty(shape, dtype=torch.int8, device=dev)
        if Tm == 0 or v is not None:
            seg.zero_(); tl.fill_(-1)
        agg = torch.zeros((1 if running else Ts,) + shape, device=dev)
        zero_rec = None if (d_gate or fused) else torch.zeros((N, 2 * C2, H, W), device=dev)
        saved = []
        t_rec = []
        v_rec = []
        recording = bool(record or v_record)
        for t in range(Tm):
            if opctx.conv_sink is not None and d_gate:
                opctx.conv_sink.sampler_spikes.append(spike)
            a_g = r_const = R = None
            g_ins = []
            if d_gate and t == 0 and fast0:
                R1, g_ins = _conv_stack_fwd(torch.zeros((1,) + shape[1:], device=dev), pg, k, packs=pk_g)
                if fused:
                    r_const = R1[0]
                else:
                    R = R1.expand(N, *R1.shape[1:]).contiguous()
            elif d_gate and fused:
                a_g = smallconv_fwd(spike, pg[0], pg[1], relu=True, out=gate_in[1][t] if keep else None, wr=pk_g[0])
                g_ins = [spike, a_g]
            elif d_gate:
                R, g_ins = _conv_stack_fwd(spike, pg, k, [gate_in[i + 1][t] for i in range(d_gate - 1)] if keep else None, packs=pk_g)
            elif not fused:
                R = zero_rec
            v_n, vs_n = torch.empty(shape, device=dev), torch.empty(shape, device=dev)
            sp_n = gate_in[0][t + 1] if keep and t + 1 < Tm else torch.empty(shape, device=dev)
            if need_grad:
                gate, vn = torch.empty(shape, device=dev), torch.empty(shape, device=dev)
                seg_b, tl_b = torch.empty_like(seg), torch.empty_like(tl)
            else:
                gate = vn = seg_b = tl_b = None
            if fused:
                _call('eas_arsnn_step_fwd', 38 * v_n.numel(), L.eas_arsnn_fused_step_fwd, ptr(A_in[t]), ptr(pk_in[1]), ptr(pin[3]), ptr(a_g),
                      ptr(pk_g[1]) if d_gate else None, ptr(pg[3]) if d_gate else None, ptr(r_const), ptr(v), ptr(vsum), ptr(seg), ptr(tl),
                      ptr(agg), ptr(v_n), ptr(vs_n), ptr(sp_n), ptr(gate), ptr(vn), ptr(seg_b), ptr(tl_b), t, Ts, 3 if running else readout,
                      int(sat), thresh, v_reset, int(soft), N, H, W, k, st)
            else:
                _call('eas_arsnn_step_fwd', 38 * v_n.numel(), L.eas_arsnn_step_fwd, ptr(X[t]), ptr(R), ptr(v), ptr(vsum), ptr(seg), ptr(tl),
                      ptr(agg), ptr(v_n), ptr(vs_n), ptr(sp_n), ptr(gate), ptr(vn), ptr(seg_b), ptr(tl_b), t, Ts, 3 if running else readout,
                      int(sat), thresh, v_reset, int(soft), N, C2, HW, st)
            if need_grad:
                saved.append((g_ins, v, vsum, gate, vn, seg_b, tl_b))
            v, vsum, spike = v_n, vs_n, sp_n
            if recording:
                if record:
                    t_rec.append(tl.to(torch.int32))
                if v_record:
                    v_rec.append(v_n[sp_n == 0])
                if not running and int(seg.min()) >= Ts:
                    recording = False
        pre_relu = None
        if running:
            out = vsum if running == 'sum' else v
        else:
            check(L.eas_arsnn_tail_fwd(ptr(v), ptr(vsum), ptr(spike), ptr(seg), ptr(tl), ptr(agg), Tm, Ts, readout, int(wz), N, C2,
                                       HW, st), 'eas_arsnn_tail_fwd')
            out = agg
        if ab:
            pre_relu = out
            out = torch.relu(out)
        ctx.cfg = cfg
        ctx.fast0 = fast0
        ctx.fused = fused
        ctx.dims = (Tm, N, Cin, C2, H, W)
        ctx.collated = bool(collated)
        ctx.saved = (saved, in_ins, spike, seg, tl, pre_relu, agg if running else None, gate_in)
        ctx.params = params
        ctx.ev_needs_grad = ctx.needs_input_grad[0]
        rec = torch.stack(t_rec) if record else None
        vrec = torch.cat(v_rec) if v_record else None
        ctx.mark_non_differentiable(*[t_ for t_ in (rec, vrec) if t_ is not None])
        return out, rec, vrec

    @staticmethod
    def backward(ctx, g_out, _g_rec=None, _g_vrec=None):
        L = _lib.lib()
        k, depth, Ts, readout, sat, wz, ab, thresh, v_reset, soft, record, running, d_in, d_gate = ctx.cfg[:14]
        Tm, N, Cin, C2, H, W = ctx.dims
        saved, in_ins, spike_last, seg, tl, pre_relu, agg, gate_in = ctx.saved
        params = ctx.params
        fused = ctx.fused
        pin, pg = params[:2 * d_in], params[2 * d_in:]
        HW = H * W
        st = stream()
        if g_out is None:
            return (None,) * (2 + len(params))
        g_out = _f32c(g_out)
        if ab:
            g_out = g_out * (pre_relu > 0)
        dev = g_out.device
        shape = (N, C2, H, W)
        jobs, slot = [], {}
        if fused and d_gate:
            wr8 = torch.empty(L.eas_smallconv_packed_floats(4, k, 8), dtype=torch.float32, device=dev)
            jobs += [(pin[2], 1, 8, 0, wr8), (pg[2], 1, 8, 4, wr8)]
        for name, w, need in (('in1', pin[2] if d_in > 1 else None, d_in > 1), ('in0', pin[0] if d_in else None, d_in and ctx.ev_needs_grad),
                              ('g1', pg[2] if d_gate > 1 else None, d_gate > 1), ('g0', pg[0] if d_gate else None, bool(d_gate))):
            if need:
                slot[name] = len(jobs)
                jobs.append((w, 1, w.shape[1], 0, None))
        pk = smallconv_pack(jobs) if jobs else []
        wr = {n: pk[i] for n, i in slot.items()}
        if running:
            g_agg = agg
            zeros = torch.zeros(shape, device=dev)
            g_v, g_vs = (zeros, g_out.contiguous()) if running == 'sum' else (g_out.contiguous(), zeros)
        else:
            g_agg = g_out
            g_v = torch.empty(shape, device=dev)
            g_vs = torch.empty(shape, device=dev)
            check(L.eas_arsnn_tail_bwd(ptr(g_agg), ptr(spike_last), ptr(seg), ptr(tl), ptr(g_v), ptr(g_vs), Tm, Ts, readout, int(wz),
                                       N, C2, HW, st), 'eas_arsnn_tail_bwd')
        g_spike = None
        gX = torch.empty((Tm, N, 2 * C2, H, W), device=dev)
        g_stage = [torch.empty((Tm, N, pg[2 * i].shape[0], H, W), device=dev) for i in range(d_gate - 1)] + ([gX] if d_gate else [])
        gA_in = torch.empty((Tm, N, 4, H, W), device=dev) if fused else None
        for t in range(Tm - 1, -1, -1):
            g_ins, v_prev, vs_prev, gate, vn, seg_b, tl_b = saved[t]
            g_vp, g_vsp = torch.empty_like(g_v), torch.empty_like(g_v)
            check(L.eas_arsnn_step_bwd(ptr(g_v), ptr(g_vs), ptr(g_spike), ptr(g_agg), ptr(v_prev), ptr(vs_prev), ptr(gate), ptr(vn),
                                       ptr(seg_b), ptr(tl_b), ptr(gX[t]), ptr(g_vp), ptr(g_vsp), t, Ts, 3 if running else readout,
                                       int(sat), thresh, v_reset, int(soft), 1.0, N, C2, HW, st), 'eas_arsnn_step_bwd')
            g_v, g_vs = g_vp, g_vsp
            if fused:
                a_in_t = in_ins[1].view(Tm, N, 4, H, W)[t]
                if d_gate and not (t == 0 and ctx.fast0) and t > 0:
                    smallconv_bwd_input_dual(gX[t], wr8, k, a_in_t, g_ins[1], gA_in[t], g_stage[0][t])
                    g_spike = smallconv_bwd_input(g_stage[0][t], pg[0], None, wr=wr['g0'])
                else:
                    smallconv_bwd_input(gX[t], pin[2], a_in_t, out=gA_in[t], wr=wr['in1'])
                    if d_gate and t == 0 and not ctx.fast0:
                        smallconv_bwd_input(gX[t], pg[2], g_ins[1], out=g_stage[0][t], wr=wr['g1'])
                    g_spike = None
                continue
            g = gX[t]
            for i in range(d_gate - 1, -1, -1):
                if t == 0 and (i == 0 or ctx.fast0):
                    break
                g = smallconv_bwd_input(g, pg[2 * i], g_ins[i] if i > 0 else None, out=g_stage[i - 1][t] if i > 0 else None,
                                        wr=wr.get('g%d' % i))
            g_spike = g if (t > 0 and d_gate) else None
        grads_g = []
        t0 = 1 if ctx.fast0 else 0
        for i in range(d_gate):
            if Tm > t0:
                gw, gb = smallconv_bwd_weight(g_stage[i][t0:].flatten(0, 1), gate_in[i][t0:].flatten(0, 1), pg[2 * i])
            else:
                gw, gb = torch.zeros_like(pg[2 * i]), torch.zeros_like(pg[2 * i + 1])
            grads_g += [gw, gb]
        if ctx.fast0:
            g1 = gX[0].sum(0, keepdim=True)
            g_ins0 = saved[0][0]
            for i in range(d_gate - 1, -1, -1):
                gw, gb = smallconv_bwd_weight(g1, g_ins0[i], pg[2 * i])
                grads_g[2 * i] = grads_g[2 * i] + gw
                grads_g[2 * i + 1] = grads_g[2 * i + 1] + gb
                if i > 0:
                    g1 = smallconv_bwd_input(g1, pg[2 * i], g_ins0[i], wr=wr['g1'])
        grads_in = [None] * (2 * d_in)
        g = gX.view(Tm * N, 2 * C2, H, W)
        for i in range(d_in - 1, -1, -1):
            grads_in[2 * i], grads_in[2 * i + 1] = smallconv_bwd_weight(g, in_ins[i], pin[2 * i], x_tm=Tm if (i == 0 and ctx.collated) else 0)
            if fused and i == 1:
                g = gA_in.view(Tm * N, 4, H, W)
            elif i > 0 or ctx.ev_needs_grad:
                g = smallconv_bwd_input(g, pin[2 * i], in_ins[i] if i > 0 else None, wr=wr.get('in%d' % i))
            else:
                g = None
        g_ev = g.view(Tm, N, Cin, H, W) if ctx.ev_needs_grad else None
        if g_ev is not None and ctx.in_collated:
            g_ev = g_ev.flip(0).transpose(0, 1)
        return (g_ev, None) + tuple(grads_in) + tuple(grads_g)


def arsnn_forward(ev_rev, input_params, gate_params, kernel_size, Ts, readout, spike_attach, write_zero, use_abs, thresh,
                  v_reset, record=False, collated=False, v_record=False):
    depth = len(input_params) // 2
    soft = v_reset is None
    cfg = (int(kernel_size), depth, int(Ts), READOUT_IDS[readout], bool(spike_attach), bool(write_zero), bool(use_abs),
           float(thresh), 0.0 if soft else float(v_reset), soft, bool(record), None, depth, len(gate_params) // 2, bool(collated), bool(v_record))
    out, rec, vrec = _ARSNNFn.apply(ev_rev, cfg, *input_params, *gate_params)
    return (out, rec, vrec) if v_record else (out, rec)


def gated_recurrence(ev_or_x, input_params, gate_params, kernel_size, readout, relu, thresh, v_reset):
    if readout not in ('sum', 'last'):
        raise NotImplementedError(readout)
    soft = v_reset is None
    d_in, d_gate = len(input_params) // 2, len(gate_params) // 2
    cfg = (int(kernel_size), max(d_in, d_gate), 1, 0, False, False, bool(relu), float(thresh), 0.0 if soft else float(v_reset), soft,
           False, readout, d_in, d_gate)
    return _ARSNNFn.apply(ev_or_x, cfg, *input_params, *gate_params)[0]


class _SmallConvFn(torch.autograd.Function):

    @staticmethod
    def forward(ctx, x, w, b, relu):
        _dev(x, w, b)
        y = smallconv_fwd(x, w, b, relu=relu)
        ctx.save_for_backward(x, w, y if relu else None)
        return y

    @staticmethod
    def backward(ctx, g):
        x, w, y = ctx.saved_tensors
        g = _f32c(g)
        if y is not None:
            g = g * (y > 0)
        gx = smallconv_bwd_input(g, w) if ctx.needs_input_grad[0] else None
        gw, gb = smallconv_bwd_weight(g, x, w)
        return gx, gw, gb, None


def small_conv_stack(x, params):
    n = len(params) // 2
    for i in range(n):
        x = _SmallConvFn.apply(x, params[2 * i], params[2 * i + 1], i < n - 1)
    return x
```

include/eas_hip.h:

```cpp
#ifndef EAS_HIP_H
#define EAS_HIP_H

#include <stdint.h>

#ifdef __cplusplus
extern "C" {
#endif

typedef void* eas_stream_t;

#define EAS_OK 0
#define EAS_ERR_INVALID_ARG (-1)
#define EAS_ERR_UNSUPPORTED (-2)
#define EAS_ERR_LAUNCH (-3)

#define EAS_SG_ATAN 0
#define EAS_SG_SIGMOID 1
#define EAS_SG_RECT 2
#define EAS_SG_PATAN 3

#define EAS_LIF_HARD_RESET 1
#define EAS_LIF_DECAY_INPUT 2
#define EAS_LIF_DETACH_RESET 4
#define EAS_LIF_FIRE_STRICT 8

int eas_abi_version(void);
void eas_kernel_trace_begin(void);
int64_t eas_kernel_trace_dump(char* buf, int64_t cap);
int64_t eas_launch_counter(void);
const char* eas_status_string(int status);

int eas_event_histogram(const uint32_t* t, const uint16_t* x, const uint16_t* y, const uint8_t* p, int64_t nev,
                        const int64_t* sample_offsets, int B, int Tm, int H, int W, int32_t* out,
                        uint32_t* oob_count, eas_stream_t stream);

int eas_event_histogram_dat(const void* records, int64_t nev, const int64_t* sample_offsets, int B, int Tm, int H, int W,
                            int32_t* out, uint32_t* oob_count, eas_stream_t stream);

int eas_counts_to_canvas(const int32_t* counts, int64_t F, int H, int W, int Hc, int Wc, float* out,
                         eas_stream_t stream);

int eas_event_frames(const uint32_t* t, const uint16_t* x, const uint16_t* y, const uint8_t* p, int64_t nev,
                     const int64_t* sample_offsets, int B, int Tm, int H, int W, int Hc, int Wc, float* frames,
                     int32_t* scratch_counts, uint32_t* oob_count, eas_stream_t stream);

int eas_counts_letterbox(const int32_t* counts, const int32_t* params, int B, int F, int H, int W, int Hc, int Wc, float* out,
                         eas_stream_t stream);

int eas_event_voxel_grid(const uint32_t* t, const uint16_t* x, const uint16_t* y, const uint8_t* p, int64_t nev,
                         const int64_t* sample_offsets, int B, int n_bins, int H, int W, double* out,
                         eas_stream_t stream);

int eas_event_voxel_cube(const uint32_t* t, const uint16_t* x, const uint16_t* y, const uint8_t* p, int64_t nev,
                         const int64_t* sample_offsets, int B, int num_slices, int tbins, int H, int W, int32_t* out,
                         eas_stream_t stream);

int eas_event_time_surface(const uint32_t* t, const uint16_t* x, const uint16_t* y, const uint8_t* p, int64_t nev,
                           const int64_t* sample_offsets, int B, int num_slices, int H, int W, double tau,
                           uint32_t* workspace, double* out, eas_stream_t stream);

int eas_event_window_search(const void* records, const int64_t* file_offsets, int F, const int32_t* file_id, const int64_t* label_t, int B,
                            int64_t window_lo, int64_t window_hi, int num_slice, int64_t* ranges, eas_stream_t stream);
int eas_event_histogram_dat_ranges(const void* records, const int64_t* ranges, int B, int Tm, int H, int W, int32_t* out,
                                   uint32_t* oob_count, eas_stream_t stream);

int eas_stacked_hist_event_sum(const uint8_t* hist, const int32_t* n_valid, int B, int Tm, int nbins, int H, int W, int Hc,
                               int Wc, float* out, eas_stream_t stream);

int eas_lif_fwd(const float* x, const float* v_in, float* v_out, const float* w_logit, float k_const, float v_th,
                float v_reset, int flags, float* spikes, float* h_save, float* mean_out, int T, int64_t M,
                eas_stream_t stream);

int eas_lif_bwd(const float* grad_s, const float* grad_mean, const float* h_save, const float* v_init,
                const float* x, const float* w_logit, float k_const, float v_th, float v_reset, int flags,
                int surrogate, float alpha, float* grad_x, float* grad_w, float* workspace, int T, int64_t M,
                eas_stream_t stream);

int64_t eas_reduce_workspace_floats(int64_t M);

int eas_lif_bwd_patan(const float* grad_s, const float* grad_mean, const float* h_save, const float* v_init,
                      const float* x, const float* w_logit, float k_const, float v_th, float v_reset, int flags,
                      const float* alpha, float* grad_alpha, float* grad_x, float* grad_w, float* workspace, int T, int64_t M,
                      eas_stream_t stream);

int eas_time_mean(const float* x, float* out, int T, int64_t M, eas_stream_t stream);
int eas_channel_sum(const float* g, float* out, int N, int C, int HW, eas_stream_t stream);


int eas_bn_stats(const float* y, int TN, int C, int HW, int replicas, float eps, float momentum, float* mean,
                 float* invstd, float* running_mean, float* running_var, double* workspace, eas_stream_t stream);
int64_t eas_bn_workspace_doubles(int C);

int eas_bn_lif_fwd(const float* y, const float* mean, const float* invstd, const float* gamma, const float* beta,
                   const float* v_in, float* v_out, const float* w_logit, float k_const, float v_th, float v_reset,
                   int flags, float* spikes, float* mean_out, int T, int N, int C, int HW, int y_bcast,
                   eas_stream_t stream);

int eas_bn_lif_bwd(const float* grad_s, const float* grad_mean, const float* y, const float* mean,
                   const float* invstd, const float* gamma, const float* beta, const float* v_init,
                   const float* w_logit, float k_const, float v_th, float v_reset, int flags, int surrogate,
                   float alpha, int batch_stats, float* grad_y, float* grad_gamma, float* grad_beta,
                   float* grad_w, double* workspace, int T, int N, int C, int HW, int y_bcast, eas_stream_t stream);

typedef struct {
    const double* partial;
    int chunks;
    int replicas;
    double count;
    float eps, momentum;
    float* running_mean;
    float* running_var;
    int pitch;
} EasBnPending;
int eas_bn_stats_partial(const float* y, int y_ctot, int TN, int C, int HW, double* workspace, eas_stream_t stream);
int eas_bn_lif_fwd_ex(const float* y, int y_ctot, float* mean, float* invstd, const float* gamma, const float* beta,
                      const float* v_in, float* v_out, const float* w_logit, float k_const, float v_th, float v_reset,
                      int flags, float* spikes, float* mean_out, int T, int N, int C, int HW, int y_bcast,
                      const EasBnPending* pending, const float* residual, int out_ctot, void* spikes_planes, const void* residual_planes,
                      int residual_ctot, eas_stream_t stream);
int eas_bn_lif_bwd_ex(const float* grad_s, int grad_s_ctot, const float* grad_mean, const float* y, int y_ctot, const float* mean,
                      const float* invstd, const float* gamma, const float* beta, const float* v_init,
                      const float* w_logit, float k_const, float v_th, float v_reset, int flags, int surrogate,
                      float alpha, int batch_stats, float* grad_y, float* grad_gamma, float* grad_beta,
                      float* grad_w, double* workspace, int T, int N, int C, int HW, int y_bcast, eas_stream_t stream);
int eas_bn_lif_bwd_patan(const float* grad_s, int grad_s_ctot, const float* grad_mean, const float* y, int y_ctot, const float* mean,
                         const float* invstd, const float* gamma, const float* beta, const float* v_init,
                         const float* w_logit, float k_const, float v_th, float v_reset, int flags, const float* alpha,
                         float* grad_alpha, int batch_stats, float* grad_y, float* grad_gamma, float* grad_beta,
                         float* grad_w, double* workspace, int T, int N, int C, int HW, int y_bcast, eas_stream_t stream);

int eas_bn_silu_fwd(const float* y, const float* mean, const float* invstd, const float* gamma, const float* beta,
                    float* out, int N, int C, int HW, eas_stream_t stream);
int eas_bn_silu_fwd_ex(const float* y, float* mean, float* invstd, const float* gamma, const float* beta,
                       float* out, int N, int C, int HW, const EasBnPending* pending, int out_ctot, int y_ctot, eas_stream_t stream);
int eas_bn_silu_bwd(const float* grad_out, const float* y, const float* mean, const float* invstd, const float* gamma,
                    const float* beta, int batch_stats, float* grad_y, float* grad_gamma, float* grad_beta,
                    double* workspace, int N, int C, int HW, int grad_out_ctot, int y_ctot, eas_stream_t stream);

int eas_arsnn_step_fwd(const float* conv_in, const float* conv_rec, const float* v, const float* vsum,
                       int8_t* seg, int8_t* t_last, float* agg, float* v_out, float* vsum_out, float* spike_out,
                       float* gate_save, float* vn_save, int8_t* seg_before, int8_t* t_last_before, int t,
                       int Ts, int readout, int spike_attach, float thresh, float v_reset, int soft_reset, int N,
                       int C2, int HW, eas_stream_t stream);

int eas_arsnn_fused_step_fwd(const float* a_in, const float* wr_in, const float* b_in, const float* a_g, const float* wr_g, const float* b_g,
                             const float* r_const, const float* v, const float* vsum, int8_t* seg, int8_t* t_last, float* agg, float* v_out,
                             float* vsum_out, float* spike_out, float* gate_save, float* vn_save, int8_t* seg_before, int8_t* t_last_before,
                             int t, int Ts, int readout, int spike_attach, float thresh, float v_reset, int soft_reset, int N, int H, int W, int k,
                             eas_stream_t stream);

int eas_arsnn_step_bwd(const float* g_v_out, const float* g_vsum_out, const float* g_spike, const float* g_agg,
                       const float* v_prev, const float* vsum_prev, const float* gate_save, const float* vn_save,
                       const int8_t* seg_before, const int8_t* t_last_before, float* g_conv, float* g_v_prev,
                       float* g_vsum_prev, int t, int Ts, int readout, int spike_attach, float thresh,
                       float v_reset, int soft_reset, float sg_alpha, int N, int C2, int HW, eas_stream_t stream);

int eas_arsnn_tail_fwd(const float* v, const float* vsum, const float* spike_last, const int8_t* seg,
                       const int8_t* t_last, float* agg, int Tm, int Ts, int readout, int write_zero, int N,
                       int C2, int HW, eas_stream_t stream);
int eas_arsnn_tail_bwd(const float* g_agg, const float* spike_last, const int8_t* seg, const int8_t* t_last,
                       float* g_v, float* g_vsum, int Tm, int Ts, int readout, int write_zero, int N, int C2,
                       int HW, eas_stream_t stream);

typedef struct {
    const float* w;
    float* wr;
    int Cin, Cout, k, mode;
    int o_total, o_off;
} EasSmallconvPackJob;
int64_t eas_smallconv_packed_floats(int n_in, int k, int o_total);
int eas_smallconv_pack_weights(const EasSmallconvPackJob* jobs, int njobs, eas_stream_t stream);
int eas_smallconv_fwd(const float* x, const float* wr, const float* b, float* y, int N, int Cin, int Cout, int H,
                      int W, int k, int relu, int x_tm, eas_stream_t stream);
int eas_smallconv_bwd_input(const float* grad_y, const float* wr, const float* relu_mask, float* grad_x, int N, int Cin,
                            int Cout, int H, int W, int k, eas_stream_t stream);
int eas_smallconv_bwd_input_dual(const float* grad_y, const float* wr, const float* mask_a, const float* mask_b, float* grad_xa,
                                 float* grad_xb, int N, int H, int W, int k, eas_stream_t stream);
int eas_smallconv_bwd_weight(const float* grad_y, const float* x, float* grad_w, float* grad_b, float* workspace,
                             int N, int Cin, int Cout, int H, int W, int k, int x_tm, eas_stream_t stream);
int64_t eas_smallconv_wgrad_workspace_floats(int Cin, int Cout, int k);

int64_t eas_conv_packed_weight_bytes(int Cout, int Cin, int ksize, int mode);
int eas_conv_pack_weights(const float* w, void* packed, int Cout, int Cin, int ksize, int mode, eas_stream_t stream);
int eas_conv_pack_weights_many(const void* jobs, int njobs, eas_stream_t stream);
int eas_conv_fwd(const float* x, const void* packed_w, const float* bias, float* y, int NI, int Cin, int Cout, int Hi,
                 int Wi, int ksize, int stride, int x_terms, int* inexact_flag, eas_stream_t stream);
int eas_conv_fwd_act(const float* x, const void* packed_w, const float* bias, float* y, int NI, int Cin, int Cout, int Hi,
                     int Wi, int ksize, int stride, int x_terms, int act, int* inexact_flag, eas_stream_t stream);
int eas_conv_fwd_stats(const float* x, const void* packed_w, float* y, int NI, int Cin, int Cout, int Hi, int Wi, int ksize, int stride,
                       int x_terms, int* inexact_flag, double* stats, int nb, eas_stream_t stream);
int eas_conv_fwd_stats_blocks(int NI, int Cin, int Cout, int Hi, int Wi, int ksize, int stride, int x_terms);
int eas_spike_planes_from_f32(const float* x, int src_ctot, void* planes, int dst_ctot, int64_t NI, int C, int HW, int* inexact_flag,
                              eas_stream_t stream);
int eas_spike_planes_to_f32(const void* planes, int src_ctot, float* x, int dst_ctot, int64_t NI, int C, int HW, eas_stream_t stream);
int eas_conv_fwd_planes(const void* x_planes, const void* packed_w, const float* bias, float* y, int NI, int Cin, int Cout, int Hi, int Wi,
                        int ksize, int stride, double* stats, int nb, eas_stream_t stream);
int eas_conv_fwd_supported(int NI, int Cin, int Cout, int Hi, int Wi, int ksize, int stride, int x_terms);
typedef struct {
    const float *gamma, *beta, *mean, *invstd;
    const float* w_logit;
    float k_const, v_th;
    void* planes;
    float* out_f32;
    int out_ctot, out_c0;
    const void* res_planes;
    const float* res_f32;
    int res_ctot;
    float* rate;
    const float* v_in;
    float* v_out;
} EasLifRange;
typedef struct {
    const void* x;
    const void* packed_w;
    int x_terms, x_shared;
    int T, N, Cin, Cout, Hi, Wi, ksize, stride;
    int csplit;
    EasLifRange range[2];
} EasConvBnLifEval;
int eas_conv_bn_lif_eval(const EasConvBnLifEval* d, eas_stream_t stream);
int eas_conv_bn_lif_eval_supported(int T, int N, int Cin, int Cout, int Hi, int Wi, int ksize, int stride, int x_terms, int x_shared);

typedef struct {
    const float *gamma, *beta, *mean, *invstd;
    float* out;
    int out_ctot, out_c0;
} EasBnActRange;
typedef struct {
    const void* x;
    const void* packed_w;
    int x_terms;
    int NI, Cin, Cout, Hi, Wi, ksize, stride;
    int act;
    int csplit;
    EasBnActRange range[2];
} EasConvBnActEval;
int eas_conv_bn_act_eval(const EasConvBnActEval* d, int* inexact_flag, eas_stream_t stream);

int eas_conv_dgrad_s2(const float* grad_y, const void* packed_w, float* grad_x, int NI, int Cin, int Cout, int Hi, int Wi,
                      eas_stream_t stream);

int eas_conv_dgrad_small_supported(int NI, int Cin, int Cout, int H, int W);
int eas_conv_dgrad_small(const float* grad_y, const float* w, float* grad_x, int NI, int Cin, int Cout, int H, int W, eas_stream_t stream);

int64_t eas_conv_wgrad_workspace_floats(int NI, int Cin, int Cout, int Hi, int Wi, int ksize, int stride, int x_terms);
int eas_conv_wgrad_parts(int NI, int Cin, int Cout, int Hi, int Wi, int stride, int x_terms);
int eas_conv_wgrad(const float* x, const float* grad_y, float* grad_w, float* workspace, int NI, int Cin, int Cout, int Hi,
                   int Wi, int ksize, int stride, int x_terms, eas_stream_t stream);
typedef struct {
    const float* slabs;
    float* grad_w;
    int n;
    int slabs_count;
} EasWgradReduceJob;
int eas_conv_wgrad_partial(const float* x, const float* grad_y, float* workspace, int NI, int Cin, int Cout, int Hi, int Wi, int ksize,
                           int stride, int x_terms, eas_stream_t stream);
int eas_conv_wgrad_planes_partial(const void* x_planes, const float* grad_y, float* workspace, int NI, int Cin, int Cout, int Hi, int Wi, int ksize,
                                  int stride, eas_stream_t stream);
int eas_conv_wgrad_reduce_many(const EasWgradReduceJob* jobs, int njobs, eas_stream_t stream);

int eas_dwconv_supported(int NI, int C, int Hi, int Wi, int stride, int x_form);
int eas_dwconv_fwd_stats_blocks(int NI, int C, int Hi, int Wi, int stride, int x_form);
int eas_dwconv_fwd(const float* x, const float* w, const float* bias, float* y, int NI, int C, int Hi, int Wi, int stride, double* stats,
                   int nb, eas_stream_t stream);
int eas_dwconv_fwd_planes(const void* x_planes, const float* w, const float* bias, float* y, int NI, int C, int Hi, int Wi, int stride,
                          double* stats, int nb, eas_stream_t stream);
int eas_dwconv_dgrad(const float* grad_y, const float* w, float* grad_x, int NI, int C, int Hi, int Wi, int stride, eas_stream_t stream);
int64_t eas_dwconv_wgrad_workspace_floats(int NI, int C, int Hi, int Wi, int stride);
int eas_dwconv_wgrad(const float* x, const float* grad_y, float* workspace, float* grad_w, int NI, int C, int Hi, int Wi, int stride,
                     eas_stream_t stream);
int eas_dwconv_wgrad_planes(const void* x_planes, const float* grad_y, float* workspace, float* grad_w, int NI, int C, int Hi, int Wi,
                            int stride, eas_stream_t stream);

int eas_spp_pool_fwd(const float* x, float* out, int64_t N, int C, int H, int W, int k0, int k1, int k2, eas_stream_t stream);
int eas_spp_pool_bwd(const float* x, const float* grad_out, float* grad_x, int64_t N, int C, int H, int W, int k0, int k1, int k2,
                     eas_stream_t stream);
int eas_spp_pool_planes_fwd(const void* x_planes, void* out_planes, int64_t N, int C, int H, int W, int k0, int k1, int k2, eas_stream_t stream);
int eas_spp_pool_planes_bwd(const void* x_planes, const float* grad_out, float* grad_x, int64_t N, int C, int H, int W, int k0, int k1, int k2,
                            eas_stream_t stream);

int64_t eas_spike_sop_workspace_doubles(void);
int eas_spike_sop(const float* x, int64_t NI, int Cin, int H, int W, int ksize, int stride, int Cout, double* out,
                  double* workspace, eas_stream_t stream);

int64_t eas_postprocess_workspace_bytes(int B, int A);
int eas_postprocess(const float* pred, int B, int A, int ncls, float conf_thre, float nms_thre, int class_agnostic, float* out,
                    int* out_count, void* workspace, eas_stream_t stream);

int eas_simota_assign(const float* grids, const float* strides, const float* gt_boxes, const float* gt_cls,
                      const unsigned char* gt_valid, const float* bbox, const float* obj, const float* cls, int B, int G, int A,
                      int nc, unsigned char* fg, long long* matched, float* matched_iou, eas_stream_t stream);

int eas_simota_assign_rows(const float* grids, const float* strides, const float* gt_boxes, const float* gt_cls,
                           const unsigned char* gt_valid, const float* dec, int B, int G, int A, int nc, unsigned char* fg,
                           long long* matched, float* matched_iou, eas_stream_t stream);

int eas_det_labels(const float* labels, int B, int G, uint8_t* gt_valid, float* gt_cls, float* gt_boxes, float* num_gts, eas_stream_t stream);
int eas_det_decode(int L, const float* const* reg, const float* const* obj, const float* const* cls, const int* hw,
                   const float* strides, int B, int nc, float* dec, eas_stream_t stream);
int eas_det_decode_eval(int L, const float* const* reg, const float* const* obj, const float* const* cls, const int* hw,
                        const float* strides, int B, int nc, float* dec, eas_stream_t stream);
int64_t eas_det_loss_workspace_doubles(void);
int eas_det_loss(int L, const float* const* reg, const float* const* obj, const float* const* cls, float* const* g_reg,
                 float* const* g_obj, float* const* g_cls, const int* hw, const float* strides, int B, int nc, const float* dec,
                 const float* gt_boxes, const float* gt_cls, int G, const unsigned char* fg, const long long* matched,
                 const float* matched_iou, const float* num_gts, int use_l1, float* out, double* workspace,
                 eas_stream_t stream);

int eas_upcat_fwd(const float* a, const float* b, float* out, int64_t M, int Ca, int Cb, int H, int W, int up, eas_stream_t stream);
int eas_upcat_bwd(const float* grad_out, float* grad_a, float* grad_b, int64_t M, int Ca, int Cb, int H, int W, int up,
                  eas_stream_t stream);
int eas_upcat_planes_fwd(const void* a_planes, const void* b_planes, void* out_planes, int64_t M, int Ca, int Cb, int H, int W, int up,
                         eas_stream_t stream);

int eas_focus(const float* src, float* dst, int64_t M, int C, int Ho, int Wo, int inverse, eas_stream_t stream);

typedef struct {
    const void* x;
    const void* packed_w;
    const float* bias;
    float* y;
    double* stats;
    int NI, Cin, Cout, Hi, Wi;
    int accumulate;
} EasConvProblem;
int eas_conv_fwd_group_plan(const EasConvProblem* problems, int n, int ksize, int x_terms, int* nb_out);
int eas_conv_fwd_group(const EasConvProblem* problems, int n, int ksize, int x_terms, eas_stream_t stream);

int eas_conv_bn_act_eval_group(const EasConvBnActEval* problems, int n, eas_stream_t stream);

typedef struct {
    const float* y;
    float* mean;
    float* invstd;
    const float* gamma;
    const float* beta;
    float* out;
    int N, C, HW, out_ctot, y_ctot;
    EasBnPending pending;
} EasBnSiluFwdProblem;
int eas_bn_silu_fwd_group(const EasBnSiluFwdProblem* problems, int n, eas_stream_t stream);
typedef struct {
    const float* grad_out;
    const float* y;
    const float* mean;
    const float* invstd;
    const float* gamma;
    const float* beta;
    float* grad_y;
    float* grad_gamma;
    float* grad_beta;
    double* workspace;
    int batch_stats, N, C, HW, grad_out_ctot, y_ctot;
} EasBnSiluBwdProblem;
int eas_bn_silu_bwd_group(const EasBnSiluBwdProblem* problems, int n, eas_stream_t stream);

typedef struct {
    const void* x;
    const float* grad_y;
    float* workspace;
    int NI, Cin, Cout, Hi, Wi;
} EasWgradProblem;
int eas_conv_wgrad_group_plan(const EasWgradProblem* problems, int n, int ksize, int x_terms, int* slabs_out);
int eas_conv_wgrad_group_partial(const EasWgradProblem* problems, int n, int ksize, int x_terms, eas_stream_t stream);

typedef struct {
    const float* g;
    float* out;
    int N, C, HW;
} EasChannelSumProblem;
int eas_channel_sum_group(const EasChannelSumProblem* problems, int n, eas_stream_t stream);

typedef struct {
    const float* gy_a;
    const float* w_a;
    int Ka;
    const float* gy_b;
    const float* w_b;
    int Kb;
    float* gx;
    int N, C, HW;
} EasPredDgradProblem;
int eas_pred_dgrad_group(const EasPredDgradProblem* problems, int n, eas_stream_t stream);

int eas_adam_table_entry_bytes(void);
int eas_adam_chunk(void);
int eas_adam_step(const void* table, int ntensors, long long total_blocks, double beta1, double beta2, double eps, eas_stream_t stream);
int eas_adam_advance_steps(const void* table, int ntensors, eas_stream_t stream);

#define EAS_ADAM_MAX_GROUPS 16
typedef struct {
    double beta1, beta2, eps;
    double group_lr[EAS_ADAM_MAX_GROUPS];
    const double* ema_updates;
    double ema_decay;
    double ema_ramp;
} EasAdamHyper;
int eas_adam_step_ex(const void* table, int ntensors, long long total_blocks, const EasAdamHyper* hyper, eas_stream_t stream);
int eas_adam_advance_steps_ex(const void* table, int ntensors, double* ema_updates, eas_stream_t stream);

int eas_cocoeval_supported(int64_t D, int64_t G, int64_t I, int K, int T, int R, int A, int M, int64_t max_gt_per_pair);
int64_t eas_cocoeval_workspace_bytes(int64_t D);
int eas_cocoeval_keys(const int32_t* det_img, const int32_t* det_cls, const float* det_score, int64_t D, const int32_t* gt_img,
                      const int32_t* gt_cls, int64_t G, int64_t I, int K, int64_t* det_key, int64_t* gt_key, eas_stream_t stream);
int eas_cocoeval_match(const int64_t* det_key, const int64_t* det_order, const float* det_box, int64_t D, const int64_t* gt_key,
                       const int64_t* gt_order, const float* gt_box, const int64_t* gt_id, int64_t G, int64_t I, int K, const double* iou_thr,
                       int T, const double* area_rng, int A, int max_det, int64_t max_gt_per_pair, int32_t* rank, uint64_t* matched,
                       uint64_t* ignored, int64_t* key2, int32_t* npig, eas_stream_t stream);
int eas_cocoeval_accumulate(const int64_t* key2, const int64_t* order2, const int32_t* rank, const uint64_t* matched, const uint64_t* ignored,
                            int64_t D, const int32_t* npig, int K, int T, const double* rec_thr, int R, int A, const int32_t* max_dets, int M,
                            double* precision, double* recall, void* workspace, eas_stream_t stream);

#ifdef __cplusplus
}
#endif
#endif
```

Measured before the change: 3437.

## Fuse ARSNN tail into last step kernels and batch small-conv weight grads

Adds last-timestep variants of the ARSNN step forward and backward kernels that fold the tail aggregation into the step, removing the separate tail kernels. It also adds a fused backward kernel that computes the gate small-conv input gradient in-kernel and feeds it straight into the step backward. A batched small-conv weight-gradient entry point replaces the per-layer calls. The aim is fewer launches and fewer intermediate tensor round-trips, at the cost of more kernel variants and env-flag complexity.

```diff
diff --git a/eas_snn_amd/_ctx.py b/eas_snn_amd/_ctx.py
--- a/eas_snn_amd/_ctx.py
+++ b/eas_snn_amd/_ctx.py
@@ -13,6 +13,9 @@
         self.fused_eval = {'1': 'all', 'all': 'all', '0': False, 'auto': 'auto'}.get(os.environ.get('EAS_FUSED_EVAL', 'auto'), 'auto')
         self.fused_ann_eval = _env_flag('EAS_FUSED_ANN_EVAL')
         self.arsnn_fused = _env_flag('EAS_ARSNN_FUSED')
+        self.arsnn_bwd_fused = _env_flag('EAS_ARSNN_BWD_FUSED')
+        self.arsnn_tails = _env_flag('EAS_ARSNN_TAILS')
+        self.smallconv_wgrad_many = _env_flag('EAS_SMALLCONV_WGRAD_MANY')
         self.small_dgrad = os.environ.get('EAS_SMALL_DGRAD', '1') != '0'
         self.defer_wgrad_reduce = _env_flag('EAS_DEFER_WGRAD_REDUCE', '0')
         self.wgrad_side_batch = int(os.environ.get('EAS_WGRAD_SIDE', '16'))
diff --git a/eas_snn_amd/_lib.py b/eas_snn_amd/_lib.py
--- a/eas_snn_amd/_lib.py
+++ b/eas_snn_amd/_lib.py
@@ -79,6 +79,11 @@
 class EasPredDgradProblem(C.Structure):
     _fields_ = [('gy_a', C.c_void_p), ('w_a', C.c_void_p), ('Ka', C.c_int), ('gy_b', C.c_void_p), ('w_b', C.c_void_p), ('Kb', C.c_int),
                 ('gx', C.c_void_p), ('N', C.c_int), ('C', C.c_int), ('HW', C.c_int)]
+
+
+class EasSmallconvWgradJob(C.Structure):
+    _fields_ = [('grad_y', C.c_void_p), ('x', C.c_void_p), ('grad_w', C.c_void_p), ('grad_b', C.c_void_p), ('N', C.c_int), ('Cin', C.c_int),
+                ('Cout', C.c_int), ('H', C.c_int), ('W', C.c_int), ('k', C.c_int), ('x_tm', C.c_int), ('add_to', C.c_int)]
 
 
 class EasAdamHyper(C.Structure):
@@ -156,6 +161,16 @@
     'eas_arsnn_tail_bwd': (C.c_int, [_P] * 6 + [C.c_int] * 7 + [_P]),
     'eas_arsnn_fused_step_fwd': (C.c_int, [_P] * 19 + [C.c_int, C.c_int, C.c_int, C.c_int, C.c_float, C.c_float, C.c_int,
                                                        C.c_int, C.c_int, C.c_int, C.c_int, _P]),
+    'eas_arsnn_step_fwd_last': (C.c_int, [_P] * 14 + [C.c_int, C.c_int, C.c_int, C.c_int, C.c_float, C.c_float, C.c_int, C.c_int,
+                                                      C.c_int, C.c_int, C.c_int, _P]),
+    'eas_arsnn_fused_step_fwd_last': (C.c_int, [_P] * 19 + [C.c_int, C.c_int, C.c_int, C.c_int, C.c_float, C.c_float, C.c_int, C.c_int,
+                                                            C.c_int, C.c_int, C.c_int, C.c_int, _P]),
+    'eas_arsnn_step_bwd_last': (C.c_int, [_P] * 10 + [C.c_int, C.c_int, C.c_int, C.c_int, C.c_float, C.c_float, C.c_int, C.c_float, C.c_int,
+                                                      C.c_int, C.c_int, C.c_int, _P]),
+    'eas_arsnn_fused_step_bwd': (C.c_int, [_P] * 14 + [C.c_int, C.c_int, C.c_int, C.c_int, C.c_float, C.c_float, C.c_int, C.c_float,
+                                                       C.c_int, C.c_int, C.c_int, C.c_int, _P]),
+    'eas_smallconv_wgrad_many_workspace_floats': (C.c_int64, [_P, C.c_int]),
+    'eas_smallconv_bwd_weight_many': (C.c_int, [_P, C.c_int, _P, _P]),
     'eas_smallconv_packed_floats': (C.c_int64, [C.c_int] * 3),
     'eas_smallconv_pack_weights': (C.c_int, [_P, C.c_int, _P]),
     'eas_smallconv_bwd_input_dual': (C.c_int, [_P] * 6 + [C.c_int] * 4 + [_P]),
diff --git a/eas_snn_amd/csrc/arsnn.hip b/eas_snn_amd/csrc/arsnn.hip
--- a/eas_snn_amd/csrc/arsnn.hip
+++ b/eas_snn_amd/csrc/arsnn.hip
@@ -19,6 +19,8 @@
     float thresh, v_reset, sg_alpha;
     int64_t plane;
     int64_t total;
+    int tail_Tm;
+    int write_zero;
 };
 
 __device__ __forceinline__ void step_elem(float g_in, float c_in, float g_rec, float c_rec, float v, float vsum,
@@ -43,6 +45,21 @@
     } else {
         vsum_out = vs1;
     }
+}
+
+__device__ __forceinline__ void tail_elem(float spike, float v_out, float vsum_out, int32_t seg, int32_t tl, float* __restrict__ agg,
+                                          int64_t i, const StepCfg& c) {
+    if (spike != 0.0f || seg >= c.Ts) return;
+    float val = c.readout == 0 ? vsum_out : (c.readout == 1 ? v_out : vsum_out / (float)(c.tail_Tm - 1 - tl));
+    if (c.write_zero) val = val * 0.0f;
+    agg[(int64_t)seg * c.total + i] += val;
+}
+
+__device__ __forceinline__ void step_tail_elem(float g_in, float c_in, float g_rec, float c_rec, float v, float vsum, int32_t& seg,
+                                               int32_t& tl, float* __restrict__ agg, int64_t i, const StepCfg& c, float& v_out,
+                                               float& vsum_out, float& spike, float& gate, float& vn) {
+    step_elem(g_in, c_in, g_rec, c_rec, v, vsum, seg, tl, agg, i, c, v_out, vsum_out, spike, gate, vn);
+    if (c.tail_Tm) tail_elem(spike, v_out, vsum_out, seg, tl, agg, i, c);
 }
 
 __global__ __launch_bounds__(EAS_BLOCK) void arsnn_step_fwd_kernel(
@@ -72,10 +89,10 @@
         if (seg_before) store_q8(seg_before + i, sg);
         if (tl_before) store_q8(tl_before + i, tl);
         float4 vo, vso, sp, ga, vn;
-        step_elem(gi.x, ci.x, gr.x, cr.x, vv.x, vs.x, sg.x, tl.x, agg, i + 0, c, vo.x, vso.x, sp.x, ga.x, vn.x);
-        step_elem(gi.y, ci.y, gr.y, cr.y, vv.y, vs.y, sg.y, tl.y, agg, i + 1, c, vo.y, vso.y, sp.y, ga.y, vn.y);
-        step_elem(gi.z, ci.z, gr.z, cr.z, vv.z, vs.z, sg.z, tl.z, agg, i + 2, c, vo.z, vso.z, sp.z, ga.z, vn.z);
-        step_elem(gi.w, ci.w, gr.w, cr.w, vv.w, vs.w, sg.w, tl.w, agg, i + 3, c, vo.w, vso.w, sp.w, ga.w, vn.w);
+        step_tail_elem(gi.x, ci.x, gr.x, cr.x, vv.x, vs.x, sg.x, tl.x, agg, i + 0, c, vo.x, vso.x, sp.x, ga.x, vn.x);
+        step_tail_elem(gi.y, ci.y, gr.y, cr.y, vv.y, vs.y, sg.y, tl.y, agg, i + 1, c, vo.y, vso.y, sp.y, ga.y, vn.y);
+        step_tail_elem(gi.z, ci.z, gr.z, cr.z, vv.z, vs.z, sg.z, tl.z, agg, i + 2, c, vo.z, vso.z, sp.z, ga.z, vn.z);
+        step_tail_elem(gi.w, ci.w, gr.w, cr.w, vv.w, vs.w, sg.w, tl.w, agg, i + 3, c, vo.w, vso.w, sp.w, ga.w, vn.w);
         *reinterpret_cast<float4*>(v_out + i) = vo;
         *reinterpret_cast<float4*>(vsum_out + i) = vso;
         *reinterpret_cast<float4*>(spike_out + i) = sp;
@@ -176,10 +193,10 @@
                 if (seg_before) store_q8(seg_before + i, sg[c2]);
                 if (tl_before) store_q8(tl_before + i, tl[c2]);
                 float4 vo, vso, sp, ga, vn;
-                step_elem(gi[0], ci[0], gr[0], cr[0], vv[c2].x, vs[c2].x, sg[c2].x, tl[c2].x, agg, i + 0, c, vo.x, vso.x, sp.x, ga.x, vn.x);
-                step_elem(gi[1], ci[1], gr[1], cr[1], vv[c2].y, vs[c2].y, sg[c2].y, tl[c2].y, agg, i + 1, c, vo.y, vso.y, sp.y, ga.y, vn.y);
-                step_elem(gi[2], ci[2], gr[2], cr[2], vv[c2].z, vs[c2].z, sg[c2].z, tl[c2].z, agg, i + 2, c, vo.z, vso.z, sp.z, ga.z, vn.z);
-                step_elem(gi[3], ci[3], gr[3], cr[3], vv[c2].w, vs[c2].w, sg[c2].w, tl[c2].w, agg, i + 3, c, vo.w, vso.w, sp.w, ga.w, vn.w);
+                step_tail_elem(gi[0], ci[0], gr[0], cr[0], vv[c2].x, vs[c2].x, sg[c2].x, tl[c2].x, agg, i + 0, c, vo.x, vso.x, sp.x, ga.x, vn.x);
+                step_tail_elem(gi[1], ci[1], gr[1], cr[1], vv[c2].y, vs[c2].y, sg[c2].y, tl[c2].y, agg, i + 1, c, vo.y, vso.y, sp.y, ga.y, vn.y);
+                step_tail_elem(gi[2], ci[2], gr[2], cr[2], vv[c2].z, vs[c2].z, sg[c2].z, tl[c2].z, agg, i + 2, c, vo.z, vso.z, sp.z, ga.z, vn.z);
+                step_tail_elem(gi[3], ci[3], gr[3], cr[3], vv[c2].w, vs[c2].w, sg[c2].w, tl[c2].w, agg, i + 3, c, vo.w, vso.w, sp.w, ga.w, vn.w);
                 *reinterpret_cast<float4*>(v_out + i) = vo;
                 *reinterpret_cast<float4*>(vsum_out + i) = vso;
                 *reinterpret_cast<float4*>(spike_out + i) = sp;
@@ -230,6 +247,19 @@
     g_gatepre = (d_vn * v_prev) * gate * (1.0f - gate);
 }
 
+__device__ __forceinline__ void tail_elem_bwd(const float* __restrict__ g_agg, int64_t i, float vn, int32_t seg_b, int32_t tl_b,
+                                              const StepCfg& c, float& gv, float& gvs) {
+    gv = 0.f;
+    gvs = 0.f;
+    const bool fired = (vn - c.thresh) > 0.0f;
+    if (!fired && seg_b < c.Ts && !c.write_zero) {
+        const float ga = g_agg[(int64_t)seg_b * c.total + i];
+        if (c.readout == 0) gvs = ga;
+        else if (c.readout == 1) gv = ga;
+        else gvs = ga / (float)(c.tail_Tm - 1 - tl_b);
+    }
+}
+
 __global__ __launch_bounds__(EAS_BLOCK) void arsnn_step_bwd_kernel(
     const float* __restrict__ g_v_out, const float* __restrict__ g_vsum_out, const float* __restrict__ g_spike,
     const float* __restrict__ g_agg, const float* __restrict__ v_prev, const float* __restrict__ vsum_prev,
@@ -241,13 +271,94 @@
         const int64_t r = i - n * c.plane;
         const int64_t cb = n * 2 * c.plane + r;
         float gg, gc, gvp, gvsp;
-        step_elem_bwd(g_v_out ? g_v_out[i] : 0.f, g_vsum_out ? g_vsum_out[i] : 0.f, g_spike ? g_spike[i] : 0.f, g_agg, i,
-                      v_prev ? v_prev[i] : 0.f, vsum_prev ? vsum_prev[i] : 0.f, gate_save[i], vn_save[i], seg_before[i], tl_before[i], c, gg, gc,
-                      gvp, gvsp);
+        const float vn = vn_save[i];
+        const int32_t sb = seg_before[i], tb = tl_before[i];
+        float gv = g_v_out ? g_v_out[i] : 0.f, gvs = g_vsum_out ? g_vsum_out[i] : 0.f;
+        if (c.tail_Tm) tail_elem_bwd(g_agg, i, vn, sb, tb, c, gv, gvs);
+        step_elem_bwd(gv, gvs, g_spike ? g_spike[i] : 0.f, g_agg, i, v_prev ? v_prev[i] : 0.f, vsum_prev ? vsum_prev[i] : 0.f, gate_save[i], vn,
+                      sb, tb, c, gg, gc, gvp, gvsp);
         g_conv[cb] = gg;
         g_conv[cb + c.plane] = gc;
         g_v_prev[i] = gvp;
         g_vsum_prev[i] = gvsp;
+    }
+}
+
+template <int K>
+__global__ __launch_bounds__(NT, 2) void arsnn_fused_step_bwd_kernel(
+    const float* __restrict__ g_stage, const float* __restrict__ wr, const float* __restrict__ g_v_out, const float* __restrict__ g_vsum_out,
+    const float* __restrict__ g_agg, const float* __restrict__ v_prev, const float* __restrict__ vsum_prev, const float* __restrict__ gate_save,
+    const float* __restrict__ vn_save, const eas_state_t* __restrict__ seg_before, const eas_state_t* __restrict__ tl_before,
+    float* __restrict__ g_conv, float* __restrict__ g_v_prev, float* __restrict__ g_vsum_prev, StepCfg c, int N, int H, int W) {
+    using SG = Stage<4, K, true>;
+    constexpr int LWF = SG::PITCH, PLANE = SG::PLANE;
+    using St = typename SG::St;
+    St st;
+    st.init(H, W);
+    __shared__ __attribute__((aligned(16))) float lds[4 * PLANE];
+    const int tiles_x = (W + TW - 1) / TW, tiles_y = (H + TH - 1) / TH;
+    const int ntiles = N * tiles_x * tiles_y;
+    const int tx = threadIdx.x & 15, ty = threadIdx.x >> 4;
+    const int HW = H * W;
+    float4 pre[St::PER];
+    unsigned okm = 0;
+    int tile = blockIdx.x;
+    if (tile < ntiles)
+        okm = st.load(g_stage, pre, tile / (tiles_x * tiles_y), H, W, ((tile / tiles_x) % tiles_y) * TH, (tile % tiles_x) * TW);
+    for (; tile < ntiles; tile += gridDim.x) {
+        const int n = tile / (tiles_x * tiles_y);
+        const int ty0 = ((tile / tiles_x) % tiles_y) * TH, tx0 = (tile % tiles_x) * TW;
+        const int nxt = tile + gridDim.x;
+        __syncthreads();
+        st.store(lds, pre, okm);
+        __syncthreads();
+        if (nxt < ntiles) okm = st.load(g_stage, pre, nxt / (tiles_x * tiles_y), H, W, ((nxt / tiles_x) % tiles_y) * TH, (nxt % tiles_x) * TW);
+        const int oy = ty0 + ty, ox = tx0 + 4 * tx;
+        const bool inside = oy < H && ox < W;
+        const int pix = oy * W + ox;
+        float4 gv[2], gvs[2], vp[2], vsp[2], ga[2], vn[2];
+        int4 sb[2], tb[2];
+#pragma unroll
+        for (int c2 = 0; c2 < 2; ++c2) {
+            gv[c2] = make_float4(0.f, 0.f, 0.f, 0.f); gvs[c2] = gv[c2]; vp[c2] = gv[c2]; vsp[c2] = gv[c2]; ga[c2] = gv[c2]; vn[c2] = gv[c2];
+            sb[c2] = make_int4(0, 0, 0, 0); tb[c2] = make_int4(-1, -1, -1, -1);
+            if (inside) {
+                const int64_t i = ((int64_t)n * 2 + c2) * HW + pix;
+                gv[c2] = *reinterpret_cast<const float4*>(g_v_out + i);
+                gvs[c2] = *reinterpret_cast<const float4*>(g_vsum_out + i);
+                if (v_prev) {
+                    vp[c2] = *reinterpret_cast<const float4*>(v_prev + i);
+                    vsp[c2] = *reinterpret_cast<const float4*>(vsum_prev + i);
+                }
+                ga[c2] = *reinterpret_cast<const float4*>(gate_save + i);
+                vn[c2] = *reinterpret_cast<const float4*>(vn_save + i);
+                sb[c2] = load_q8(seg_before + i);
+                tb[c2] = load_q8(tl_before + i);
+            }
+        }
+        __builtin_amdgcn_sched_barrier(0);
+        f2 acc[4][1];
+#pragma unroll
+        for (int j = 0; j < 4; ++j) acc[j][0] = f2{0.f, 0.f};
+        sc_accumulate<4, 2, K, LWF, SG::NQ, SG::OFS>(lds, PLANE, wr, acc, tx, ty);
+        if (inside) {
+#pragma unroll
+            for (int c2 = 0; c2 < 2; ++c2) {
+                const int64_t i = ((int64_t)n * 2 + c2) * HW + pix;
+                float gs[4];
+#pragma unroll
+                for (int j = 0; j < 4; ++j) gs[j] = c2 ? acc[j][0].y : acc[j][0].x;
+                float4 gg, gc, gvp, gvsp;
+                step_elem_bwd(gv[c2].x, gvs[c2].x, gs[0], g_agg, i + 0, vp[c2].x, vsp[c2].x, ga[c2].x, vn[c2].x, sb[c2].x, tb[c2].x, c, gg.x, gc.x, gvp.x, gvsp.x);
+                step_elem_bwd(gv[c2].y, gvs[c2].y, gs[1], g_agg, i + 1, vp[c2].y, vsp[c2].y, ga[c2].y, vn[c2].y, sb[c2].y, tb[c2].y, c, gg.y, gc.y, gvp.y, gvsp.y);
+                step_elem_bwd(gv[c2].z, gvs[c2].z, gs[2], g_agg, i + 2, vp[c2].z, vsp[c2].z, ga[c2].z, vn[c2].z, sb[c2].z, tb[c2].z, c, gg.z, gc.z, gvp.z, gvsp.z);
+                step_elem_bwd(gv[c2].w, gvs[c2].w, gs[3], g_agg, i + 3, vp[c2].w, vsp[c2].w, ga[c2].w, vn[c2].w, sb[c2].w, tb[c2].w, c, gg.w, gc.w, gvp.w, gvsp.w);
+                *reinterpret_cast<float4*>(g_conv + ((int64_t)n * 4 + c2) * HW + pix) = gg;
+                *reinterpret_cast<float4*>(g_conv + ((int64_t)n * 4 + 2 + c2) * HW + pix) = gc;
+                *reinterpret_cast<float4*>(g_v_prev + i) = gvp;
+                *reinterpret_cast<float4*>(g_vsum_prev + i) = gvsp;
+            }
+        }
     }
 }
 
@@ -290,11 +401,11 @@
 
 extern "C" {
 
-int eas_arsnn_step_fwd(const float* conv_in, const float* conv_rec, const float* v, const float* vsum,
-                       int8_t* seg, int8_t* t_last, float* agg, float* v_out, float* vsum_out, float* spike_out,
-                       float* gate_save, float* vn_save, int8_t* seg_before, int8_t* t_last_before, int t,
-                       int Ts, int readout, int spike_attach, float thresh, float v_reset, int soft_reset, int N,
-                       int C2, int HW, eas_stream_t stream) {
+static int step_fwd(const float* conv_in, const float* conv_rec, const float* v, const float* vsum,
+                    int8_t* seg, int8_t* t_last, float* agg, float* v_out, float* vsum_out, float* spike_out,
+                    float* gate_save, float* vn_save, int8_t* seg_before, int8_t* t_last_before, int t,
+                    int Ts, int readout, int spike_attach, float thresh, float v_reset, int soft_reset, int tail_Tm, int write_zero, int N,
+                    int C2, int HW, eas_stream_t stream) {
     if (!conv_in || !conv_rec || (v == nullptr) != (vsum == nullptr) || !seg || !t_last || !agg || !v_out || !vsum_out || !spike_out)
         return EAS_ERR_INVALID_ARG;
     if (N < 1 || C2 < 1 || HW < 1 || Ts < 1 || t < 0 || readout < 0 || readout > 3) return EAS_ERR_INVALID_ARG;
@@ -303,7 +414,7 @@
          (uintptr_t)v_out | (uintptr_t)vsum_out | (uintptr_t)spike_out | (uintptr_t)gate_save | (uintptr_t)vn_save |
          (uintptr_t)seg_before | (uintptr_t)t_last_before) & 15)
         return EAS_ERR_INVALID_ARG;
-    StepCfg c{t, Ts, readout, spike_attach, soft_reset, thresh, v_reset, 1.0f, (int64_t)C2 * HW, (int64_t)N * C2 * HW};
+    StepCfg c{t, Ts, readout, spike_attach, soft_reset, thresh, v_reset, 1.0f, (int64_t)C2 * HW, (int64_t)N * C2 * HW, tail_Tm, write_zero};
     EAS_CLEAR_ERR();
     EAS_LAUNCH(arsnn_step_fwd_kernel, dim3(eas_grid_1d(c.total / VEC)), dim3(EAS_BLOCK), 0, eas_s(stream), conv_in,
                        conv_rec, v, vsum, seg, t_last, agg, v_out, vsum_out, spike_out, gate_save, vn_save, seg_before,
@@ -312,11 +423,30 @@
     return EAS_OK;
 }
 
-int eas_arsnn_fused_step_fwd(const float* a_in, const float* wr_in, const float* b_in, const float* a_g, const float* wr_g, const float* b_g,
-                             const float* r_const, const float* v, const float* vsum, int8_t* seg, int8_t* t_last, float* agg, float* v_out,
-                             float* vsum_out, float* spike_out, float* gate_save, float* vn_save, int8_t* seg_before, int8_t* t_last_before,
-                             int t, int Ts, int readout, int spike_attach, float thresh, float v_reset, int soft_reset, int N, int H, int W, int k,
-                             eas_stream_t stream) {
+int eas_arsnn_step_fwd(const float* conv_in, const float* conv_rec, const float* v, const float* vsum,
+                       int8_t* seg, int8_t* t_last, float* agg, float* v_out, float* vsum_out, float* spike_out,
+                       float* gate_save, float* vn_save, int8_t* seg_before, int8_t* t_last_before, int t,
+                       int Ts, int readout, int spike_attach, float thresh, float v_reset, int soft_reset, int N,
+                       int C2, int HW, eas_stream_t stream) {
+    return step_fwd(conv_in, conv_rec, v, vsum, seg, t_last, agg, v_out, vsum_out, spike_out, gate_save, vn_save, seg_before, t_last_before, t,
+                    Ts, readout, spike_attach, thresh, v_reset, soft_reset, 0, 0, N, C2, HW, stream);
+}
+
+int eas_arsnn_step_fwd_last(const float* conv_in, const float* conv_rec, const float* v, const float* vsum,
+                            int8_t* seg, int8_t* t_last, float* agg, float* v_out, float* vsum_out, float* spike_out,
+                            float* gate_save, float* vn_save, int8_t* seg_before, int8_t* t_last_before, int Tm,
+                            int Ts, int readout, int spike_attach, float thresh, float v_reset, int soft_reset, int write_zero,
+                            int N, int C2, int HW, eas_stream_t stream) {
+    if (Tm < 1 || readout > 2) return EAS_ERR_INVALID_ARG;
+    return step_fwd(conv_in, conv_rec, v, vsum, seg, t_last, agg, v_out, vsum_out, spike_out, gate_save, vn_save, seg_before, t_last_before,
+                    Tm - 1, Ts, readout, spike_attach, thresh, v_reset, soft_reset, Tm, write_zero != 0, N, C2, HW, stream);
+}
+
+static int fused_step_fwd(const float* a_in, const float* wr_in, const float* b_in, const float* a_g, const float* wr_g, const float* b_g,
+                          const float* r_const, const float* v, const float* vsum, int8_t* seg, int8_t* t_last, float* agg, float* v_out,
+                          float* vsum_out, float* spike_out, float* gate_save, float* vn_save, int8_t* seg_before, int8_t* t_last_before,
+                          int t, int Ts, int readout, int spike_attach, float thresh, float v_reset, int soft_reset, int tail_Tm, int write_zero,
+                          int N, int H, int W, int k, eas_stream_t stream) {
     if (!a_in || !wr_in || (a_g && !wr_g) || (v == nullptr) != (vsum == nullptr) || !seg || !t_last || !agg || !v_out || !vsum_out || !spike_out)
         return EAS_ERR_INVALID_ARG;
     if (N < 1 || H < 1 || W < 1 || Ts < 1 || t < 0 || readout < 0 || readout > 3) return EAS_ERR_INVALID_ARG;
@@ -326,7 +456,7 @@
          (uintptr_t)t_last_before) & 15)
         return EAS_ERR_INVALID_ARG;
     const int HW = H * W;
-    StepCfg c{t, Ts, readout, spike_attach, soft_reset, thresh, v_reset, 1.0f, (int64_t)2 * HW, (int64_t)N * 2 * HW};
+    StepCfg c{t, Ts, readout, spike_attach, soft_reset, thresh, v_reset, 1.0f, (int64_t)2 * HW, (int64_t)N * 2 * HW, tail_Tm, write_zero};
     int tiles = N * ((H + TH - 1) / TH) * ((W + TW - 1) / TW);
     if (tiles > 256 * 6) tiles = 256 * 6;
     hipStream_t st = eas_s(stream);
@@ -350,18 +480,38 @@
     return EAS_OK;
 }
 
-int eas_arsnn_step_bwd(const float* g_v_out, const float* g_vsum_out, const float* g_spike, const float* g_agg,
-                       const float* v_prev, const float* vsum_prev, const float* gate_save, const float* vn_save,
-                       const int8_t* seg_before, const int8_t* t_last_before, float* g_conv, float* g_v_prev,
-                       float* g_vsum_prev, int t, int Ts, int readout, int spike_attach, float thresh,
-                       float v_reset, int soft_reset, float sg_alpha, int N, int C2, int HW, eas_stream_t stream) {
+int eas_arsnn_fused_step_fwd(const float* a_in, const float* wr_in, const float* b_in, const float* a_g, const float* wr_g, const float* b_g,
+                             const float* r_const, const float* v, const float* vsum, int8_t* seg, int8_t* t_last, float* agg, float* v_out,
+                             float* vsum_out, float* spike_out, float* gate_save, float* vn_save, int8_t* seg_before, int8_t* t_last_before,
+                             int t, int Ts, int readout, int spike_attach, float thresh, float v_reset, int soft_reset, int N, int H, int W, int k,
+                             eas_stream_t stream) {
+    return fused_step_fwd(a_in, wr_in, b_in, a_g, wr_g, b_g, r_const, v, vsum, seg, t_last, agg, v_out, vsum_out, spike_out, gate_save, vn_save,
+                          seg_before, t_last_before, t, Ts, readout, spike_attach, thresh, v_reset, soft_reset, 0, 0, N, H, W, k, stream);
+}
+
+int eas_arsnn_fused_step_fwd_last(const float* a_in, const float* wr_in, const float* b_in, const float* a_g, const float* wr_g,
+                                  const float* b_g, const float* r_const, const float* v, const float* vsum, int8_t* seg, int8_t* t_last,
+                                  float* agg, float* v_out, float* vsum_out, float* spike_out, float* gate_save, float* vn_save,
+                                  int8_t* seg_before, int8_t* t_last_before, int Tm, int Ts, int readout, int spike_attach, float thresh,
+                                  float v_reset, int soft_reset, int write_zero, int N, int H, int W, int k, eas_stream_t stream) {
+    if (Tm < 1 || readout > 2) return EAS_ERR_INVALID_ARG;
+    return fused_step_fwd(a_in, wr_in, b_in, a_g, wr_g, b_g, r_const, v, vsum, seg, t_last, agg, v_out, vsum_out, spike_out, gate_save, vn_save,
+                          seg_before, t_last_before, Tm - 1, Ts, readout, spike_attach, thresh, v_reset, soft_reset, Tm, write_zero != 0, N, H, W,
+                          k, stream);
+}
+
+static int step_bwd(const float* g_v_out, const float* g_vsum_out, const float* g_spike, const float* g_agg,
+                    const float* v_prev, const float* vsum_prev, const float* gate_save, const float* vn_save,
+                    const int8_t* seg_before, const int8_t* t_last_before, float* g_conv, float* g_v_prev,
+                    float* g_vsum_prev, int t, int Ts, int readout, int spike_attach, float thresh,
+                    float v_reset, int soft_reset, float sg_alpha, int tail_Tm, int write_zero, int N, int C2, int HW, eas_stream_t stream) {
     if (!g_agg || (v_prev == nullptr) != (vsum_prev == nullptr) || !gate_save || !vn_save || !seg_before || !t_last_before || !g_conv ||
         !g_v_prev || !g_vsum_prev)
         return EAS_ERR_INVALID_ARG;
     if (N < 1 || C2 < 1 || HW < 1 || Ts < 1 || t < 0 || readout < 0 || readout > 3 || !(sg_alpha > 0.f))
         return EAS_ERR_INVALID_ARG;
     StepCfg c{t, Ts, readout, spike_attach, soft_reset, thresh, v_reset, sg_alpha, (int64_t)C2 * HW,
-              (int64_t)N * C2 * HW};
+              (int64_t)N * C2 * HW, tail_Tm, write_zero};
     EAS_CLEAR_ERR();
     EAS_LAUNCH(arsnn_step_bwd_kernel, dim3(eas_grid_1d(c.total)), dim3(EAS_BLOCK), 0, eas_s(stream), g_v_out,
                        g_vsum_out, g_spike, g_agg, v_prev, vsum_prev, gate_save, vn_save, seg_before, t_last_before, g_conv,
@@ -370,6 +520,55 @@
     return EAS_OK;
 }
 
+int eas_arsnn_step_bwd(const float* g_v_out, const float* g_vsum_out, const float* g_spike, const float* g_agg,
+                       const float* v_prev, const float* vsum_prev, const float* gate_save, const float* vn_save,
+                       const int8_t* seg_before, const int8_t* t_last_before, float* g_conv, float* g_v_prev,
+                       float* g_vsum_prev, int t, int Ts, int readout, int spike_attach, float thresh,
+                       float v_reset, int soft_reset, float sg_alpha, int N, int C2, int HW, eas_stream_t stream) {
+    return step_bwd(g_v_out, g_vsum_out, g_spike, g_agg, v_prev, vsum_prev, gate_save, vn_save, seg_before, t_last_before, g_conv, g_v_prev,
+                    g_vsum_prev, t, Ts, readout, spike_attach, thresh, v_reset, soft_reset, sg_alpha, 0, 0, N, C2, HW, stream);
+}
+
+int eas_arsnn_step_bwd_last(const float* g_agg, const float* v_prev, const float* vsum_prev, const float* gate_save,
+                            const float* vn_save, const int8_t* seg_before, const int8_t* t_last_before, float* g_conv,
+                            float* g_v_prev, float* g_vsum_prev, int Tm, int Ts, int readout, int spike_attach, float thresh,
+                            float v_reset, int soft_reset, float sg_alpha, int write_zero, int N, int C2, int HW, eas_stream_t stream) {
+    if (Tm < 1 || readout > 2) return EAS_ERR_INVALID_ARG;
+    return step_bwd(nullptr, nullptr, nullptr, g_agg, v_prev, vsum_prev, gate_save, vn_save, seg_before, t_last_before, g_conv, g_v_prev,
+                    g_vsum_prev, Tm - 1, Ts, readout, spike_attach, thresh, v_reset, soft_reset, sg_alpha, Tm, write_zero != 0, N, C2, HW, stream);
+}
+
+int eas_arsnn_fused_step_bwd(const float* g_stage, const float* wr, const float* g_v_out, const float* g_vsum_out, const float* g_agg,
+                             const float* v_prev, const float* vsum_prev, const float* gate_save, const float* vn_save,
+                             const int8_t* seg_before, const int8_t* t_last_before, float* g_conv, float* g_v_prev, float* g_vsum_prev,
+                             int t, int Ts, int readout, int spike_attach, float thresh, float v_reset, int soft_reset, float sg_alpha,
+                             int N, int H, int W, int k, eas_stream_t stream) {
+    if (!g_stage || !wr || !g_v_out || !g_vsum_out || !g_agg || (v_prev == nullptr) != (vsum_prev == nullptr) || !gate_save || !vn_save ||
+        !seg_before || !t_last_before || !g_conv || !g_v_prev || !g_vsum_prev)
+        return EAS_ERR_INVALID_ARG;
+    if (N < 1 || H < 1 || W < 1 || Ts < 1 || t < 0 || readout < 0 || readout > 3 || !(sg_alpha > 0.f)) return EAS_ERR_INVALID_ARG;
+    if (W % 4 != 0 || (k != 3 && k != 5 && k != 7)) return EAS_ERR_UNSUPPORTED;
+    if (((uintptr_t)g_stage | (uintptr_t)wr | (uintptr_t)g_v_out | (uintptr_t)g_vsum_out | (uintptr_t)v_prev | (uintptr_t)vsum_prev |
+         (uintptr_t)gate_save | (uintptr_t)vn_save | (uintptr_t)seg_before | (uintptr_t)t_last_before | (uintptr_t)g_conv | (uintptr_t)g_v_prev |
+         (uintptr_t)g_vsum_prev) & 15)
+        return EAS_ERR_INVALID_ARG;
+    const int HW = H * W;
+    StepCfg c{t, Ts, readout, spike_attach, soft_reset, thresh, v_reset, sg_alpha, (int64_t)2 * HW, (int64_t)N * 2 * HW, 0, 0};
+    int tiles = N * ((H + TH - 1) / TH) * ((W + TW - 1) / TW);
+    if (tiles > 256 * 6) tiles = 256 * 6;
+    hipStream_t st = eas_s(stream);
+    EAS_CLEAR_ERR();
+#define EAS_FUSED_BWD(K_)                                                                                                              \
+    EAS_LAUNCH((arsnn_fused_step_bwd_kernel<K_>), dim3(tiles), dim3(NT), 0, st, g_stage, wr, g_v_out, g_vsum_out, g_agg, v_prev,       \
+               vsum_prev, gate_save, vn_save, seg_before, t_last_before, g_conv, g_v_prev, g_vsum_prev, c, N, H, W)
+    if (k == 3) EAS_FUSED_BWD(3);
+    else if (k == 5) EAS_FUSED_BWD(5);
+    else EAS_FUSED_BWD(7);
+#undef EAS_FUSED_BWD
+    EAS_CHECK_LAUNCH();
+    return EAS_OK;
+}
+
 int eas_arsnn_tail_fwd(const float* v, const float* vsum, const float* spike_last, const int8_t* seg,
                        const int8_t* t_last, float* agg, int Tm, int Ts, int readout, int write_zero, int N,
                        int C2, int HW, eas_stream_t stream) {
diff --git a/eas_snn_amd/csrc/smallconv_wgrad_mfma.hip b/eas_snn_amd/csrc/smallconv_wgrad_mfma.hip
--- a/eas_snn_amd/csrc/smallconv_wgrad_mfma.hip
+++ b/eas_snn_amd/csrc/smallconv_wgrad_mfma.hip
@@ -74,8 +74,8 @@
 }
 
 template <int CIN, int COUT, int K, bool VEC>
-__global__ __launch_bounds__(VEC ? 4 * NTH : NTH) void smallconv_wgrad_mfma_kernel(const float* __restrict__ gy, const float* __restrict__ x,
-                                                                                   float* __restrict__ partial, int N, int H, int W, int x_tm) {
+__device__ __forceinline__ void sw_block(const float* __restrict__ gy, const float* __restrict__ x, float* __restrict__ partial, int N, int H,
+                                         int W, int x_tm, unsigned char* smem, const int bidx, const int G) {
     using S = Sw<CIN, COUT, K>;
     const int xS = x_tm ? N / x_tm : 0;
     auto x_img = [&](int n) {
@@ -85,7 +85,6 @@
     };
     constexpr int PAD = S::PAD;
     constexpr int NBUF = VEC ? 2 : 1;
-    extern __shared__ __attribute__((aligned(16))) unsigned char smem[];
     const int tid = threadIdx.x, lane = tid & 63;
     constexpr int NTS = VEC ? 2 * NTH : NTH;
     constexpr int NCW = VEC ? 2 * NWV : NWV;
@@ -259,9 +258,8 @@
                 sw_store_terms<1, 9>(dst + S::X_COPY, S::X_TERM, v);
             }
         };
-        const int G = gridDim.x;
         const bool stager = __builtin_amdgcn_readfirstlane(tid >> 6) < NTS / 64;
-        int t = blockIdx.x;
+        int t = bidx;
         if (stager) {
             Pre pa, pb;
             issue(pa, t);
@@ -301,7 +299,7 @@
         }
     } else {
         __syncthreads();
-        for (int t = blockIdx.x; t < ntiles; t += gridDim.x) {
+        for (int t = bidx; t < ntiles; t += G) {
             int n, h0, w0;
             tile_origin(t, n, h0, w0);
             for (int id = tid; id < S::G_ITEMS; id += NTH) {
@@ -349,9 +347,108 @@
         float s = 0.f;
 #pragma unroll
         for (int wv = 0; wv < NCW; ++wv) s += red[(wv * 32 + m) * 33 + nn];
-        partial[(int64_t)blockIdx.x * S::NOUT + e] = s;
-    }
-}
+        partial[(int64_t)bidx * S::NOUT + e] = s;
+    }
+}
+
+template <int CIN, int COUT, int K, bool VEC>
+__global__ __launch_bounds__(VEC ? 4 * NTH : NTH) void smallconv_wgrad_mfma_kernel(const float* __restrict__ gy, const float* __restrict__ x,
+                                                                                   float* __restrict__ partial, int N, int H, int W, int x_tm) {
+    extern __shared__ __attribute__((aligned(16))) unsigned char smem[];
+    sw_block<CIN, COUT, K, VEC>(gy, x, partial, N, H, W, x_tm, smem, blockIdx.x, gridDim.x);
+}
+
+constexpr int kManyJobs = 8;
+struct WgradJobs {
+    const float* gy[kManyJobs];
+    const float* x[kManyJobs];
+    float* partial[kManyJobs];
+    int N[kManyJobs], Cin[kManyJobs], H[kManyJobs], W[kManyJobs], x_tm[kManyJobs], G[kManyJobs];
+    int njobs;
+};
+
+template <int K>
+__global__ __launch_bounds__(4 * NTH) void smallconv_wgrad_many_kernel(const WgradJobs jobs) {
+    extern __shared__ __attribute__((aligned(16))) unsigned char smem[];
+    const int b = blockIdx.x;
+    for (int j = 0; j < jobs.njobs; ++j) {
+        const int G = jobs.G[j];
+        if (b >= G) continue;
+        __syncthreads();
+        if (jobs.Cin[j] == 4) sw_block<4, 4, K, true>(jobs.gy[j], jobs.x[j], jobs.partial[j], jobs.N[j], jobs.H[j], jobs.W[j], jobs.x_tm[j], smem, b, G);
+        else sw_block<2, 4, K, true>(jobs.gy[j], jobs.x[j], jobs.partial[j], jobs.N[j], jobs.H[j], jobs.W[j], jobs.x_tm[j], smem, b, G);
+    }
+}
+
+struct WgradFin {
+    const float* partial[kManyJobs];
+    float* gw[kManyJobs];
+    float* gb[kManyJobs];
+    int nblocks[kManyJobs], nout[kManyJobs], nw[kManyJobs], add_to[kManyJobs], first[kManyJobs + 1];
+    int njobs;
+};
+
+__device__ __forceinline__ double sw_fin_sum(const float* __restrict__ partial, int nblocks, int nout, int e) {
+    double s = 0.0;
+    for (int b = threadIdx.x; b < nblocks; b += EAS_WAVE) s += (double)partial[(int64_t)b * nout + e];
+    return eas_wave_sum(s);
+}
+
+__global__ __launch_bounds__(EAS_WAVE) void smallconv_wgrad_many_finalize(const WgradFin f) {
+    int j = 0;
+    while (j + 1 < f.njobs && (int)blockIdx.x >= f.first[j + 1]) ++j;
+    const int e = blockIdx.x - f.first[j];
+    float r = (float)sw_fin_sum(f.partial[j], f.nblocks[j], f.nout[j], e);
+    for (int a = j + 1; a < f.njobs; ++a)
+        if (f.add_to[a] == j) r = r + (float)sw_fin_sum(f.partial[a], f.nblocks[a], f.nout[a], e);
+    if (threadIdx.x == 0) {
+        if (e < f.nw[j]) f.gw[j][e] = r;
+        else if (f.gb[j]) f.gb[j][e - f.nw[j]] = r;
+    }
+}
+
+template <int K>
+int sw_launch_many(const WgradJobs& jobs, int grid, int lds_bytes, hipStream_t st) {
+    auto kern = smallconv_wgrad_many_kernel<K>;
+    static bool attr_set = false;
+    if (!attr_set) {
+        if (hipFuncSetAttribute((const void*)kern, hipFuncAttributeMaxDynamicSharedMemorySize, 160 * 1024) != hipSuccess) return EAS_ERR_LAUNCH;
+        attr_set = true;
+    }
+    EAS_LAUNCH(kern, dim3(grid), dim3(4 * NTH), lds_bytes, st, jobs);
+    return EAS_OK;
+}
+
+template <int K>
+int sw_stage_bytes(int Cin, int Cout) {
+    if (Cin == 4 && Cout == 4) return Sw<4, 4, K>::STAGE_BYTES;
+    if (Cin == 2 && Cout == 4) return Sw<2, 4, K>::STAGE_BYTES;
+    return -1;
+}
+
+int64_t sw_many_tiles(const EasSmallconvWgradJob& q) { return (int64_t)q.N * ((q.H + RB - 1) / RB) * ((q.W + WC - 1) / WC); }
+
+int sw_many_check(const EasSmallconvWgradJob* jobs, int njobs) {
+    if (!jobs || njobs < 1 || njobs > kManyJobs) return EAS_ERR_INVALID_ARG;
+    for (int j = 0; j < njobs; ++j) {
+        const EasSmallconvWgradJob& q = jobs[j];
+        if (!q.grad_y || !q.x || q.N < 1 || q.H < 1 || q.W < 1 || q.x_tm < 0 || (q.x_tm > 0 && q.N % q.x_tm != 0)) return EAS_ERR_INVALID_ARG;
+        if (q.add_to >= j) return EAS_ERR_INVALID_ARG;
+        if (q.add_to >= 0) {
+            const EasSmallconvWgradJob& t = jobs[q.add_to];
+            if (t.add_to >= 0 || t.Cin != q.Cin || t.Cout != q.Cout || t.k != q.k) return EAS_ERR_INVALID_ARG;
+        } else if (!q.grad_w) {
+            return EAS_ERR_INVALID_ARG;
+        }
+        if (q.k != jobs[0].k || (q.k != 5 && q.k != 7)) return EAS_ERR_UNSUPPORTED;
+        if (sw_stage_bytes<5>(q.Cin, q.Cout) < 0) return EAS_ERR_UNSUPPORTED;
+        if ((q.W & 3) != 0 || ((((uintptr_t)q.grad_y) | ((uintptr_t)q.x)) & 15) != 0) return EAS_ERR_UNSUPPORTED;
+        if (sw_many_tiles(q) > 0x7fffffff) return EAS_ERR_UNSUPPORTED;
+    }
+    return EAS_OK;
+}
+
+constexpr int kManyBlocks = 256;
 
 template <int CIN, int COUT, int K>
 int sw_launch_k(bool vec, const float* gy, const float* x, float* partial, int nblocks, int N, int H, int W, int x_tm, hipStream_t st) {
@@ -400,3 +497,50 @@
     else return EAS_ERR_UNSUPPORTED;
     return rc;
 }
+
+extern "C" {
+
+int64_t eas_smallconv_wgrad_many_workspace_floats(const EasSmallconvWgradJob* jobs, int njobs) {
+    if (sw_many_check(jobs, njobs) != EAS_OK) return 0;
+    int64_t n = 0;
+    for (int j = 0; j < njobs; ++j) n += (int64_t)kManyBlocks * ((int64_t)jobs[j].Cout * jobs[j].Cin * jobs[j].k * jobs[j].k + jobs[j].Cout);
+    return n;
+}
+
+int eas_smallconv_bwd_weight_many(const EasSmallconvWgradJob* jobs, int njobs, float* workspace, eas_stream_t stream) {
+    const int rc = sw_many_check(jobs, njobs);
+    if (rc != EAS_OK) return rc;
+    if (!workspace || ((uintptr_t)workspace & 15)) return EAS_ERR_INVALID_ARG;
+    WgradJobs wj{};
+    WgradFin wf{};
+    const int k = jobs[0].k;
+    int grid = 0, lds = 0, nfin = 0;
+    int64_t off = 0;
+    for (int j = 0; j < njobs; ++j) {
+        const EasSmallconvWgradJob& q = jobs[j];
+        const int64_t tiles = sw_many_tiles(q);
+        const int G = tiles < kManyBlocks ? (int)tiles : kManyBlocks;
+        const int nw = q.Cout * q.Cin * k * k, nout = nw + q.Cout;
+        wj.gy[j] = q.grad_y; wj.x[j] = q.x; wj.partial[j] = workspace + off;
+        wj.N[j] = q.N; wj.Cin[j] = q.Cin; wj.H[j] = q.H; wj.W[j] = q.W; wj.x_tm[j] = q.x_tm; wj.G[j] = G;
+        wf.partial[j] = workspace + off; wf.gw[j] = q.grad_w; wf.gb[j] = q.grad_b;
+        wf.nblocks[j] = G; wf.nout[j] = nout; wf.nw[j] = nw; wf.add_to[j] = q.add_to;
+        wf.first[j] = nfin;
+        if (q.add_to < 0) nfin += nout;
+        off += (int64_t)kManyBlocks * nout;
+        if (G > grid) grid = G;
+        const int sb = 2 * (k == 5 ? sw_stage_bytes<5>(q.Cin, q.Cout) : sw_stage_bytes<7>(q.Cin, q.Cout));
+        if (sb > lds) lds = sb;
+    }
+    wj.njobs = njobs; wf.njobs = njobs; wf.first[njobs] = nfin;
+    hipStream_t st = eas_s(stream);
+    EAS_CLEAR_ERR();
+    const int lrc = k == 5 ? sw_launch_many<5>(wj, grid, lds, st) : sw_launch_many<7>(wj, grid, lds, st);
+    if (lrc != EAS_OK) return lrc;
+    EAS_CHECK_LAUNCH();
+    EAS_LAUNCH(smallconv_wgrad_many_finalize, dim3(nfin), dim3(EAS_WAVE), 0, st, wf);
+    EAS_CHECK_LAUNCH();
+    return EAS_OK;
+}
+
+}
diff --git a/eas_snn_amd/ops.py b/eas_snn_amd/ops.py
--- a/eas_snn_amd/ops.py
+++ b/eas_snn_amd/ops.py
@@ -19,7 +19,8 @@
     '_STATE_WRITEBACK': 'state_writeback', '_TIMER': 'timer', '_TAG': 'tag', '_CALL_LOG': 'call_log', 'SPIKE_PLANES': 'spike_planes',
     '_PLANES_SCOPE': 'planes_scope', '_INVSTD_SCOPE': 'invstd_scope', 'CONV_STATS': 'conv_stats', 'CONV_STATS_MAX_BLOCKS': 'conv_stats_max_blocks',
     '_WANT_CONV_STATS': 'want_conv_stats', '_CONV_STATS_SLOT': 'conv_stats_slot', 'FUSED_EVAL': 'fused_eval', '_REPLICAS': 'replicas',
-    'ARSNN_FUSED': 'arsnn_fused', 'DEFER_WGRAD_REDUCE': 'defer_wgrad_reduce', '_PENDING_REDUCE': 'pending_reduce',
+    'ARSNN_FUSED': 'arsnn_fused', 'ARSNN_BWD_FUSED': 'arsnn_bwd_fused', 'ARSNN_TAILS': 'arsnn_tails', 'SMALLCONV_WGRAD_MANY': 'smallconv_wgrad_many',
+    'DEFER_WGRAD_REDUCE': 'defer_wgrad_reduce', '_PENDING_REDUCE': 'pending_reduce',
     'WGRAD_SIDE_BATCH': 'wgrad_side_batch', '_SIDE': 'side',
     'VERIFY_SMALL_INT': 'verify_small_int', 'SMALL_DGRAD': 'small_dgrad', '_PACK_SCOPE': 'pack_scope', '_PACK_GEN': 'pack_gen', '_FROZEN': 'frozen',
     '_CONV_SINK': 'conv_sink', 'FUSED_ANN_EVAL': 'fused_ann_eval', '_DEFERRED': 'deferred_counters', 'DWCONV': 'dwconv',
diff --git a/eas_snn_amd/ops_sampler.py b/eas_snn_amd/ops_sampler.py
--- a/eas_snn_amd/ops_sampler.py
+++ b/eas_snn_amd/ops_sampler.py
@@ -73,6 +73,42 @@
     return gw, gb
 
 
+def smallconv_bwd_weight_many(jobs):
+    L = _lib.lib()
+    prep = []
+    for gy, x, w, x_tm, add_to in jobs:
+        gy, x = _f32c(gy), _f32c(x)
+        assert x.numel() == gy.shape[0] * w.shape[1] * gy.shape[2] * gy.shape[3] and (not x_tm or (x.dim() == 5 and x.shape[1] == x_tm))
+        assert add_to is None or (0 <= add_to < len(prep) and prep[add_to][4] < 0 and prep[add_to][2].shape == w.shape)
+        prep.append((gy, x, w, int(x_tm), -1 if add_to is None else int(add_to)))
+    form = os.environ.get('EAS_SW_FORM', '')
+    k = prep[0][2].shape[-1] if prep else 0
+    walk = (opctx.smallconv_wgrad_many and 0 < len(prep) <= 8 and k in (5, 7) and (not form or form[0] == 'm')
+            and all(w.shape[-1] == k and w.shape[0] == 4 and w.shape[1] in (2, 4) and gy.shape[3] % 4 == 0 and gy.data_ptr() % 16 == 0
+                    and x.data_ptr() % 16 == 0 for gy, x, w, _, _ in prep))
+    outs = []
+    if not walk:
+        for gy, x, w, x_tm, add_to in prep:
+            gw, gb = smallconv_bwd_weight(gy, x, w, x_tm=x_tm)
+            if add_to >= 0:
+                outs[add_to] = (outs[add_to][0] + gw, outs[add_to][1] + gb)
+            outs.append(None if add_to >= 0 else (gw, gb))
+        return outs
+    arr = (_lib.EasSmallconvWgradJob * len(prep))()
+    nbytes = 0
+    for j, (gy, x, w, x_tm, add_to) in enumerate(prep):
+        N, Cout, H, W = gy.shape
+        gw = gb = None
+        if add_to < 0:
+            gw, gb = torch.empty_like(w), torch.empty(Cout, dtype=torch.float32, device=gy.device)
+        outs.append(None if add_to >= 0 else (gw, gb))
+        arr[j] = _lib.EasSmallconvWgradJob(gy.data_ptr(), x.data_ptr(), ptr(gw), ptr(gb), N, w.shape[1], Cout, H, W, k, x_tm, add_to)
+        nbytes += 4 * (gy.numel() + x.numel())
+    ws = torch.empty(L.eas_smallconv_wgrad_many_workspace_floats(arr, len(prep)), dtype=torch.float32, device=prep[0][0].device)
+    _call('eas_smallconv_bwd_weight', nbytes, L.eas_smallconv_bwd_weight_many, arr, len(prep), ptr(ws), stream())
+    return outs
+
+
 def _conv_stack_fwd(x, params, k, mids=None, packs=None):
     ins = []
     n = len(params) // 2
@@ -81,7 +117,6 @@
         x = smallconv_fwd(x, params[2 * i], params[2 * i + 1], relu=(i < n - 1), out=mids[i] if mids is not None and i < n - 1 else None,
                           wr=packs[i] if packs is not None else None)
     return x, ins
-
 
 
 
@@ -157,6 +192,7 @@
         saved = []
         t_rec = []
         v_rec = []
+        tails = bool(opctx.arsnn_tails and not running and Tm > 0)
         recording = bool(record or v_record)
         for t in range(Tm):
             if opctx.conv_sink is not None and d_gate:
@@ -183,11 +219,21 @@
                 seg_b, tl_b = torch.empty_like(seg), torch.empty_like(tl)
             else:
                 gate = vn = seg_b = tl_b = None
-            if fused:
+            last = tails and t == Tm - 1
+            if fused and last:
+                _call('eas_arsnn_step_fwd', 38 * v_n.numel(), L.eas_arsnn_fused_step_fwd_last, ptr(A_in[t]), ptr(pk_in[1]), ptr(pin[3]), ptr(a_g),
+                      ptr(pk_g[1]) if d_gate else None, ptr(pg[3]) if d_gate else None, ptr(r_const), ptr(v), ptr(vsum), ptr(seg), ptr(tl),
+                      ptr(agg), ptr(v_n), ptr(vs_n), ptr(sp_n), ptr(gate), ptr(vn), ptr(seg_b), ptr(tl_b), Tm, Ts, readout,
+                      int(sat), thresh, v_reset, int(soft), int(wz), N, H, W, k, st)
+            elif fused:
                 _call('eas_arsnn_step_fwd', 38 * v_n.numel(), L.eas_arsnn_fused_step_fwd, ptr(A_in[t]), ptr(pk_in[1]), ptr(pin[3]), ptr(a_g),
                       ptr(pk_g[1]) if d_gate else None, ptr(pg[3]) if d_gate else None, ptr(r_const), ptr(v), ptr(vsum), ptr(seg), ptr(tl),
                       ptr(agg), ptr(v_n), ptr(vs_n), ptr(sp_n), ptr(gate), ptr(vn), ptr(seg_b), ptr(tl_b), t, Ts, 3 if running else readout,
                       int(sat), thresh, v_reset, int(soft), N, H, W, k, st)
+            elif last:
+                _call('eas_arsnn_step_fwd', 38 * v_n.numel(), L.eas_arsnn_step_fwd_last, ptr(X[t]), ptr(R), ptr(v), ptr(vsum), ptr(seg), ptr(tl),
+                      ptr(agg), ptr(v_n), ptr(vs_n), ptr(sp_n), ptr(gate), ptr(vn), ptr(seg_b), ptr(tl_b), Tm, Ts, readout,
+                      int(sat), thresh, v_reset, int(soft), int(wz), N, C2, HW, st)
             else:
                 _call('eas_arsnn_step_fwd', 38 * v_n.numel(), L.eas_arsnn_step_fwd, ptr(X[t]), ptr(R), ptr(v), ptr(vsum), ptr(seg), ptr(tl),
                       ptr(agg), ptr(v_n), ptr(vs_n), ptr(sp_n), ptr(gate), ptr(vn), ptr(seg_b), ptr(tl_b), t, Ts, 3 if running else readout,
@@ -206,8 +252,9 @@
         if running:
             out = vsum if running == 'sum' else v
         else:
-            check(L.eas_arsnn_tail_fwd(ptr(v), ptr(vsum), ptr(spike), ptr(seg), ptr(tl), ptr(agg), Tm, Ts, readout, int(wz), N, C2,
-                                       HW, st), 'eas_arsnn_tail_fwd')
+            if not tails:
+                check(L.eas_arsnn_tail_fwd(ptr(v), ptr(vsum), ptr(spike), ptr(seg), ptr(tl), ptr(agg), Tm, Ts, readout, int(wz), N, C2,
+                                           HW, st), 'eas_arsnn_tail_fwd')
             out = agg
         if ab:
             pre_relu = out
@@ -215,6 +262,7 @@
         ctx.cfg = cfg
         ctx.fast0 = fast0
         ctx.fused = fused
+        ctx.tails = tails
         ctx.dims = (Tm, N, Cin, C2, H, W)
         ctx.collated = bool(collated)
         ctx.saved = (saved, in_ins, spike, seg, tl, pre_relu, agg if running else None, gate_in)
@@ -258,6 +306,9 @@
             g_agg = agg
             zeros = torch.zeros(shape, device=dev)
             g_v, g_vs = (zeros, g_out.contiguous()) if running == 'sum' else (g_out.contiguous(), zeros)
+        elif ctx.tails:
+            g_agg = g_out
+            g_v = g_vs = None
         else:
             g_agg = g_out
             g_v = torch.empty(shape, device=dev)
@@ -265,21 +316,31 @@
             check(L.eas_arsnn_tail_bwd(ptr(g_agg), ptr(spike_last), ptr(seg), ptr(tl), ptr(g_v), ptr(g_vs), Tm, Ts, readout, int(wz),
                                        N, C2, HW, st), 'eas_arsnn_tail_bwd')
         g_spike = None
+        bwd_fused = bool(opctx.arsnn_bwd_fused and fused and d_gate)
         gX = torch.empty((Tm, N, 2 * C2, H, W), device=dev)
         g_stage = [torch.empty((Tm, N, pg[2 * i].shape[0], H, W), device=dev) for i in range(d_gate - 1)] + ([gX] if d_gate else [])
         gA_in = torch.empty((Tm, N, 4, H, W), device=dev) if fused else None
         for t in range(Tm - 1, -1, -1):
             g_ins, v_prev, vs_prev, gate, vn, seg_b, tl_b = saved[t]
-            g_vp, g_vsp = torch.empty_like(g_v), torch.empty_like(g_v)
-            check(L.eas_arsnn_step_bwd(ptr(g_v), ptr(g_vs), ptr(g_spike), ptr(g_agg), ptr(v_prev), ptr(vs_prev), ptr(gate), ptr(vn),
-                                       ptr(seg_b), ptr(tl_b), ptr(gX[t]), ptr(g_vp), ptr(g_vsp), t, Ts, 3 if running else readout,
-                                       int(sat), thresh, v_reset, int(soft), 1.0, N, C2, HW, st), 'eas_arsnn_step_bwd')
+            g_vp, g_vsp = torch.empty(shape, device=dev), torch.empty(shape, device=dev)
+            if t == Tm - 1 and g_v is None:
+                check(L.eas_arsnn_step_bwd_last(ptr(g_agg), ptr(v_prev), ptr(vs_prev), ptr(gate), ptr(vn), ptr(seg_b), ptr(tl_b), ptr(gX[t]),
+                                                ptr(g_vp), ptr(g_vsp), Tm, Ts, readout, int(sat), thresh, v_reset, int(soft), 1.0, int(wz),
+                                                N, C2, HW, st), 'eas_arsnn_step_bwd_last')
+            elif bwd_fused and t < Tm - 1:
+                _call('eas_arsnn_step_bwd', 100 * N * HW, L.eas_arsnn_fused_step_bwd, ptr(g_stage[0][t + 1]), ptr(wr['g0']), ptr(g_v), ptr(g_vs),
+                      ptr(g_agg), ptr(v_prev), ptr(vs_prev), ptr(gate), ptr(vn), ptr(seg_b), ptr(tl_b), ptr(gX[t]), ptr(g_vp), ptr(g_vsp), t, Ts,
+                      3 if running else readout, int(sat), thresh, v_reset, int(soft), 1.0, N, H, W, k, st)
+            else:
+                check(L.eas_arsnn_step_bwd(ptr(g_v), ptr(g_vs), ptr(g_spike), ptr(g_agg), ptr(v_prev), ptr(vs_prev), ptr(gate), ptr(vn),
+                                           ptr(seg_b), ptr(tl_b), ptr(gX[t]), ptr(g_vp), ptr(g_vsp), t, Ts, 3 if running else readout,
+                                           int(sat), thresh, v_reset, int(soft), 1.0, N, C2, HW, st), 'eas_arsnn_step_bwd')
             g_v, g_vs = g_vp, g_vsp
             if fused:
                 a_in_t = in_ins[1].view(Tm, N, 4, H, W)[t]
                 if d_gate and not (t == 0 and ctx.fast0) and t > 0:
                     smallconv_bwd_input_dual(gX[t], wr8, k, a_in_t, g_ins[1], gA_in[t], g_stage[0][t])
-                    g_spike = smallconv_bwd_input(g_stage[0][t], pg[0], None, wr=wr['g0'])
+                    g_spike = None if bwd_fused else smallconv_bwd_input(g_stage[0][t], pg[0], None, wr=wr['g0'])
                 else:
                     smallconv_bwd_input(gX[t], pin[2], a_in_t, out=gA_in[t], wr=wr['in1'])
                     if d_gate and t == 0 and not ctx.fast0:
@@ -293,33 +354,43 @@
                 g = smallconv_bwd_input(g, pg[2 * i], g_ins[i] if i > 0 else None, out=g_stage[i - 1][t] if i > 0 else None,
                                         wr=wr.get('g%d' % i))
             g_spike = g if (t > 0 and d_gate) else None
-        grads_g = []
+        jobs, at_g, at_g0, at_in = [], {}, {}, {}
         t0 = 1 if ctx.fast0 else 0
         for i in range(d_gate):
             if Tm > t0:
-                gw, gb = smallconv_bwd_weight(g_stage[i][t0:].flatten(0, 1), gate_in[i][t0:].flatten(0, 1), pg[2 * i])
-            else:
-                gw, gb = torch.zeros_like(pg[2 * i]), torch.zeros_like(pg[2 * i + 1])
-            grads_g += [gw, gb]
+                at_g[i] = len(jobs)
+                jobs.append((g_stage[i][t0:].flatten(0, 1), gate_in[i][t0:].flatten(0, 1), pg[2 * i], 0, None))
         if ctx.fast0:
             g1 = gX[0].sum(0, keepdim=True)
             g_ins0 = saved[0][0]
             for i in range(d_gate - 1, -1, -1):
-                gw, gb = smallconv_bwd_weight(g1, g_ins0[i], pg[2 * i])
-                grads_g[2 * i] = grads_g[2 * i] + gw
-                grads_g[2 * i + 1] = grads_g[2 * i + 1] + gb
+                at_g0[i] = len(jobs)
+                jobs.append((g1, g_ins0[i], pg[2 * i], 0, at_g.get(i)))
                 if i > 0:
                     g1 = smallconv_bwd_input(g1, pg[2 * i], g_ins0[i], wr=wr['g1'])
-        grads_in = [None] * (2 * d_in)
         g = gX.view(Tm * N, 2 * C2, H, W)
         for i in range(d_in - 1, -1, -1):
-            grads_in[2 * i], grads_in[2 * i + 1] = smallconv_bwd_weight(g, in_ins[i], pin[2 * i], x_tm=Tm if (i == 0 and ctx.collated) else 0)
+            at_in[i] = len(jobs)
+            jobs.append((g, in_ins[i], pin[2 * i], Tm if (i == 0 and ctx.collated) else 0, None))
             if fused and i == 1:
                 g = gA_in.view(Tm * N, 4, H, W)
             elif i > 0 or ctx.ev_needs_grad:
                 g = smallconv_bwd_input(g, pin[2 * i], in_ins[i] if i > 0 else None, wr=wr.get('in%d' % i))
             else:
                 g = None
+        res = smallconv_bwd_weight_many(jobs) if jobs else []
+        grads_g = []
+        for i in range(d_gate):
+            if i in at_g:
+                gw, gb = res[at_g[i]]
+            else:
+                gw, gb = torch.zeros_like(pg[2 * i]), torch.zeros_like(pg[2 * i + 1])
+                if i in at_g0:
+                    gw, gb = gw + res[at_g0[i]][0], gb + res[at_g0[i]][1]
+            grads_g += [gw, gb]
+        grads_in = [None] * (2 * d_in)
+        for i in range(d_in):
+            grads_in[2 * i], grads_in[2 * i + 1] = res[at_in[i]]
         g_ev = g.view(Tm, N, Cin, H, W) if ctx.ev_needs_grad else None
         if g_ev is not None and ctx.in_collated:
             g_ev = g_ev.flip(0).transpose(0, 1)
diff --git a/include/eas_hip.h b/include/eas_hip.h
--- a/include/eas_hip.h
+++ b/include/eas_hip.h
@@ -155,6 +155,26 @@
                        float* g_vsum_prev, int t, int Ts, int readout, int spike_attach, float thresh,
                        float v_reset, int soft_reset, float sg_alpha, int N, int C2, int HW, eas_stream_t stream);
 
+int eas_arsnn_step_fwd_last(const float* conv_in, const float* conv_rec, const float* v, const float* vsum,
+                            int8_t* seg, int8_t* t_last, float* agg, float* v_out, float* vsum_out, float* spike_out,
+                            float* gate_save, float* vn_save, int8_t* seg_before, int8_t* t_last_before, int Tm,
+                            int Ts, int readout, int spike_attach, float thresh, float v_reset, int soft_reset, int write_zero,
+                            int N, int C2, int HW, eas_stream_t stream);
+int eas_arsnn_fused_step_fwd_last(const float* a_in, const float* wr_in, const float* b_in, const float* a_g, const float* wr_g,
+                                  const float* b_g, const float* r_const, const float* v, const float* vsum, int8_t* seg, int8_t* t_last,
+                                  float* agg, float* v_out, float* vsum_out, float* spike_out, float* gate_save, float* vn_save,
+                                  int8_t* seg_before, int8_t* t_last_before, int Tm, int Ts, int readout, int spike_attach, float thresh,
+                                  float v_reset, int soft_reset, int write_zero, int N, int H, int W, int k, eas_stream_t stream);
+int eas_arsnn_step_bwd_last(const float* g_agg, const float* v_prev, const float* vsum_prev, const float* gate_save,
+                            const float* vn_save, const int8_t* seg_before, const int8_t* t_last_before, float* g_conv,
+                            float* g_v_prev, float* g_vsum_prev, int Tm, int Ts, int readout, int spike_attach, float thresh,
+                            float v_reset, int soft_reset, float sg_alpha, int write_zero, int N, int C2, int HW, eas_stream_t stream);
+int eas_arsnn_fused_step_bwd(const float* g_stage, const float* wr, const float* g_v_out, const float* g_vsum_out, const float* g_agg,
+                             const float* v_prev, const float* vsum_prev, const float* gate_save, const float* vn_save,
+                             const int8_t* seg_before, const int8_t* t_last_before, float* g_conv, float* g_v_prev, float* g_vsum_prev,
+                             int t, int Ts, int readout, int spike_attach, float thresh, float v_reset, int soft_reset, float sg_alpha,
+                             int N, int H, int W, int k, eas_stream_t stream);
+
 int eas_arsnn_tail_fwd(const float* v, const float* vsum, const float* spike_last, const int8_t* seg,
                        const int8_t* t_last, float* agg, int Tm, int Ts, int readout, int write_zero, int N,
                        int C2, int HW, eas_stream_t stream);
@@ -179,6 +199,16 @@
 int eas_smallconv_bwd_weight(const float* grad_y, const float* x, float* grad_w, float* grad_b, float* workspace,
                              int N, int Cin, int Cout, int H, int W, int k, int x_tm, eas_stream_t stream);
 int64_t eas_smallconv_wgrad_workspace_floats(int Cin, int Cout, int k);
+typedef struct {
+    const float* grad_y;
+    const float* x;
+    float* grad_w;
+    float* grad_b;
+    int N, Cin, Cout, H, W, k, x_tm;
+    int add_to;
+} EasSmallconvWgradJob;
+int64_t eas_smallconv_wgrad_many_workspace_floats(const EasSmallconvWgradJob* jobs, int njobs);
+int eas_smallconv_bwd_weight_many(const EasSmallconvWgradJob* jobs, int njobs, float* workspace, eas_stream_t stream);
 
 int64_t eas_conv_packed_weight_bytes(int Cout, int Cin, int ksize, int mode);
 int eas_conv_pack_weights(const float* w, void* packed, int Cout, int Cin, int ksize, int mode, eas_stream_t stream);
```

Result: no change. 3463, median of 6 (+0.7%).
